# Lecanyu/SparsifyPoseGraph

Hardware: AMD Instinct MI355X
Metric: nodes_marginalized_per_s (higher is better)
Workload: dtype f64

## Files before the change

sparsifyposegraph_amd/csrc/spg_graph_impl.h:

```cpp
#pragma once
#include <algorithm>
#include <atomic>
#include <chrono>
#include <cmath>
#include <cstdio>
#include <cstdlib>
#include <cstring>
#include <set>
#include <string>
#include <thread>
#if defined(__linux__)
#include <pthread.h>
#include <sched.h>
#endif
#include <unistd.h>
#include <unordered_map>
#include <unordered_set>
#include <vector>
#include "../../include/spg.h"
#include "spg_internal.h"

namespace {
inline int pose_stride(int d) { return d == 3 ? 3 : 7; }
inline int info_len(int d) { return d * (d + 1) / 2; }
inline double now_s() {
    return std::chrono::duration<double>(std::chrono::steady_clock::now().time_since_epoch()).count();
}
inline int64_t align_up(int64_t x, int64_t a) { return (x + a - 1) / a * a; }
inline void cpu_pause() {
#if defined(__x86_64__)
    __builtin_ia32_pause();
#endif
}
inline void spin_wait(uint32_t &spins) {
    if (++spins > 4096) std::this_thread::yield();
    else cpu_pause();
}
}

struct HostMirror {
    double *p = nullptr;
    size_t n = 0, cap = 0;
    ~HostMirror() { free(p); }
    HostMirror() {}
    HostMirror(const HostMirror &) = delete;
    HostMirror &operator=(const HostMirror &) = delete;
    double *data() { return p; }
    const double *data() const { return p; }
    size_t size() const { return n; }
    double &operator[](size_t i) { return p[i]; }
    const double &operator[](size_t i) const { return p[i]; }
    void resize(size_t m) {
        if (m > cap) {
            size_t nc = std::max(m, cap * 2);
            p = (double *)realloc(p, nc * sizeof(double));
            if (!p) abort();
            cap = nc;
        }
        n = m;
    }
};

template <class T, int N>
struct InlVec {
    int32_t n = 0, cap = N;
    union { T inl[N]; T *ptr; };
    InlVec() {}
    InlVec(const InlVec &o) : n(o.n), cap(o.cap) {
        if (cap > N) { ptr = (T *)malloc(sizeof(T) * (size_t)cap); memcpy(ptr, o.ptr, sizeof(T) * (size_t)n); }
        else memcpy(inl, o.inl, sizeof inl);
    }
    InlVec(InlVec &&o) noexcept : n(o.n), cap(o.cap) {
        if (cap > N) { ptr = o.ptr; o.cap = N; o.n = 0; }
        else memcpy(inl, o.inl, sizeof inl);
    }
    InlVec &operator=(InlVec o) noexcept {
        if (cap > N) free(ptr);
        n = o.n; cap = o.cap;
        if (cap > N) { ptr = o.ptr; o.cap = N; o.n = 0; }
        else memcpy(inl, o.inl, sizeof inl);
        return *this;
    }
    ~InlVec() { if (cap > N) free(ptr); }
    T *data() { return cap > N ? ptr : inl; }
    const T *data() const { return cap > N ? ptr : inl; }
    T *begin() { return data(); }
    T *end() { return data() + n; }
    const T *begin() const { return data(); }
    const T *end() const { return data() + n; }
    size_t size() const { return (size_t)n; }
    bool empty() const { return n == 0; }
    T &operator[](size_t i) { return data()[i]; }
    const T &operator[](size_t i) const { return data()[i]; }
    T &back() { return data()[n - 1]; }
    void pop_back() { n--; }
    void clear() { n = 0; }
    void push_back(const T &v) {
        if (n == cap) {
            int32_t nc = cap * 2;
            T *p = (T *)malloc(sizeof(T) * (size_t)nc);
            if (!p) abort();
            memcpy(p, data(), sizeof(T) * (size_t)n);
            if (cap > N) free(ptr);
            ptr = p; cap = nc;
        }
        data()[n++] = v;
    }
};

struct spg_ctx {
    spg_backend be{};
    bool is_hip = false;
    int rank = 0, nranks = 1;
    void *rccl = nullptr;
    int tag_counter = 0;
    int linear_solver = 0;
    double pcg_rel_tol = 0;
    int pcg_max_iter = 0;
    spg_pcg_stats pcg_stats{};
    spg::StreamPort *sim_port = nullptr;
    char err[768] = {0};
};

struct GEdge {
    int64_t off;
    int64_t key;
    int32_t len;
    int32_t vtx[2];
    int16_t nv;
    int8_t kind;
    uint8_t alive;
};

struct RoundBlanket {
    int32_t root;
    int32_t n_remove;
    int32_t vbeg = 0, nv = 0;
    int32_t ebeg = 0, ne = 0;
    int32_t rank = 0;
    int32_t owner = -1;
    spg_blanket_desc desc{};
};

struct BlanketLog { int32_t root_id, round, status, info; double kld, min_gap; };

struct Batch {
    std::vector<RoundBlanket> rb;
    std::vector<int32_t> rb_verts, rb_edges;
    std::vector<spg_blanket_desc> h_blk;
    std::vector<int64_t> h_vpo;
    std::vector<spg_edge_ref> h_er;
    std::vector<int32_t> h_ev;
    std::vector<int64_t> chunk_hdr;
    spg_round_info rinfo{};
    bool round_open = false;
    bool used_mailbox = false;
    int eff_ranks = 1, eff_rank = 0;
    int slot = 0;
    int seq = 0;
    int round_no = 0;
    int tag = 0;
    double t_launch = 0;
    std::vector<std::pair<int32_t, int64_t>> kld_pending;
    alignas(64) std::atomic<int> submitted{1};
    int submit_rc = 0;
    char pad_[56];
};

struct OwnRefT { int32_t oid; uint32_t gen; };

struct spg_graph {
    spg_ctx *ctx = nullptr;
    int d = 0, ps = 0, rec = 0;
    std::vector<int32_t> vid;
    std::unordered_map<int32_t, int32_t> vidx;
    std::vector<int32_t> vdirect;
    bool vdirect_ok = true;
    int32_t index_of(int32_t id) const {
        if (vdirect_ok) return (id >= 0 && (size_t)id < vdirect.size()) ? vdirect[(size_t)id] : -1;
        auto it = vidx.find(id);
        return it == vidx.end() ? -1 : it->second;
    }
    std::vector<uint8_t> valive;
    std::vector<int64_t> vpose;
    struct AdjEnt { int32_t eid, other; operator int32_t() const { return eid; } };
    struct SVtx {
        int32_t nown;
        int32_t own[4];
        int32_t slot;
    };
    struct alignas(64) VRec {
        InlVec<AdjEnt, 7> adj;
        SVtx s;
        int32_t id, pad_;
        int64_t pose;
        char spare_[24];
        VRec() { s.nown = 0; s.slot = -1; id = 0; pad_ = 0; pose = 0; }
    };
    std::vector<VRec> vr;
    std::vector<InlVec<struct OwnRefT, 3>> vown;
    std::vector<int32_t> cst;
    std::vector<GEdge> edges;
    std::vector<int32_t> everts;
    int n_live_v = 0, n_live_e = 0;
    void *dev = nullptr;
    int64_t cap = 0, used = 0;
    HostMirror host;
    int64_t dev_synced = 0;
    int64_t stale_lo = 0, stale_hi = 0;
    bool active = false;
    spg_options opts{};
    int rank = 0, nranks = 1;
    std::vector<int32_t> pending;
    size_t pend_head = 0;
    std::vector<uint8_t> in_set;
    static constexpr int NB = 8;
    Batch bt[NB];
    Batch *B = &bt[0];
    struct Owner { int32_t batch, off, len; uint32_t gen; };
    using OwnRef = OwnRefT;
    std::vector<Owner> owners;
    std::vector<int32_t> owner_free, transient;
    std::vector<int32_t> Dpool;
    int shard_threshold = -1;
    int round_no = 0, launch_seq = 0;
    bool pipelined = false;
    spg_marg_stats stats{};
    double tr_age = 0, tr_wait = 0, tr_first = 0; long tr_n = 0;
    std::vector<BlanketLog> log;
    std::vector<double> hdr_buf;
    std::thread sub_thread;
    static constexpr uint32_t SUBQ = 8;
    bool sub_active = false;
    struct alignas(64) SubShared {
        alignas(64) std::atomic<uint32_t> tail{0};
        alignas(64) Batch *q[SUBQ] = {nullptr};
        alignas(64) std::atomic<uint32_t> head{0};
        alignas(64) double seconds = 0;
        alignas(64) std::atomic<bool> run{false};
        char pad_[64];
    } sub;
    std::vector<int32_t> live_rank;
    long n_mutations = 0, live_rank_stamp = -1;
    int64_t next_key = 0, key_base = 0;
    static constexpr int64_t kKeyStride = 65536;
    std::vector<int32_t> lpos;
    std::vector<int32_t> vstamp, estamp;
    int32_t stamp = 0;
    std::vector<int32_t> ocnt;
    std::vector<int32_t> lidx;
    std::vector<int32_t> s_newpending, s_B, s_centres, s_Dv, s_tmp, s_work, s_seen, s_hit, s_vix;
    std::vector<double> s_cost;
    std::vector<int> s_first;
    static constexpr int kSOwn = 4, kSMaxV = 16, kSMaxE = 44;
    struct SSlot {
        int32_t pos, root, nv, ne, n_new_max, tag, logi, bell;
        int32_t launched;
        int32_t npend, pend[3];
        int32_t mcell;
        int64_t new_off, out_off;
        int32_t verts[kSMaxV];
        int32_t edges[kSMaxE];
    };
    std::vector<SSlot> sslots;
    std::vector<int32_t> s_free, s_fifo, s_fin, s_woken, s_ready, wl_next, wl_stable, wl_done;
    int64_t unsorted_from = -1;
    bool layout_diverged = false;
    int stream_emulation = -1;
    int stream_disabled = 0;
    int robust_kind = 0, robust_gap = 1;
    double robust_delta = 1.0;
};

static inline const int32_t *edge_verts(const spg_graph *g, const GEdge &e) {
    return e.nv == 2 ? e.vtx : g->everts.data() + e.vtx[0];
}

inline int set_err(spg_ctx *c, int code, const char *fmt, const char *a = "") {
    if (c) snprintf(c->err, sizeof c->err, fmt, a);
    return code;
}

int sync_host(spg_graph *g);
int sync_device(spg_graph *g);
void canonicalize_edge_order(spg_graph *g);
#pragma GCC visibility push(hidden)
int arena_ensure(spg_graph *g, int64_t need);
int add_edge_idx(spg_graph *g, int kind, int nv, const int32_t *vix, int64_t off, int32_t len, int64_t key = -1);
void pose_compose(int d, const double *a, const double *b, double *o);
void pose_inverse(int d, const double *a, double *o);
void quiesce_submission(spg_graph *g);
int stream_marginalize(spg_graph *g, bool *started = nullptr);
#pragma GCC visibility pop

namespace {
inline void next_stamp(spg_graph *g) {
    if (g->vstamp.size() < g->vid.size()) g->vstamp.resize(g->vid.size(), 0);
    if (g->estamp.size() < g->edges.size()) g->estamp.resize(g->edges.size(), 0);
    g->stamp++;
}

inline void mark_stale(spg_graph *g, int64_t lo, int64_t hi) {
    if (g->stale_hi <= g->stale_lo) { g->stale_lo = lo; g->stale_hi = hi; }
    else { g->stale_lo = std::min(g->stale_lo, lo); g->stale_hi = std::max(g->stale_hi, hi); }
}

inline void copy_backend_error(spg_ctx *c) { snprintf(c->err, sizeof c->err, "%s", spg::hip_backend_error(&c->be)); }

enum MailState { MAIL_NOT_YET = 0, MAIL_READY = 1, MAIL_FINAL = 2 };
inline MailState mail_state(double word, double tag) {
    return word == SPG_READY_WORD(tag) ? MAIL_READY : word == SPG_FINAL_WORD(tag) ? MAIL_FINAL : MAIL_NOT_YET;
}

inline bool out_record_well_formed(const double *rec, const spg_blanket_desc &bd, int nv) {
    const int n_new = (int)rec[4];
    if (n_new < 0 || n_new > bd.n_new_max) return false;
    int vsum = 0;
    for (int e = 0; e < n_new; e++) {
        const double nvd = rec[SPG_OUT_HDR + 4 * e + 3], reld = rec[SPG_OUT_HDR + 4 * e + 1], lend = rec[SPG_OUT_HDR + 4 * e + 2];
        if (!(nvd >= 1 && nvd <= nv && reld >= 0 && lend >= 1 && reld + lend <= (double)bd.new_len)) return false;
        for (int i = 0; i < (int)nvd; i++) { const double li = rec[SPG_OUT_HDR + 4 * bd.n_new_max + vsum + i]; if (!(li >= 0 && li < nv)) return false; }
        vsum += (int)nvd;
        if (vsum > bd.n_new_vert_max) return false;
    }
    return true;
}
template <class F>
inline void for_each_new_edge(const double *rec, int n_new, int n_new_max, F &&fn) {
    const double *lv = rec + SPG_OUT_HDR + 4 * n_new_max;
    for (int e = 0; e < n_new; e++) {
        const double *t = rec + SPG_OUT_HDR + 4 * e;
        const int nv = (int)t[3];
        fn(e, (int)t[0], (int64_t)t[1], (int32_t)t[2], nv, lv);
        lv += nv;
    }
}
template <class F>
inline void for_each_compact_edge(const double *rec, int n_new, F &&fn) {
    uint64_t w[2];
    memcpy(w, rec + 6, 16);
    for (int e = 0; e < n_new; e++) {
        const unsigned pr = (unsigned)(w[e >> 3] >> (8 * (e & 7))) & 0xffu;
        fn(e, (int)(pr & 15u), (int)(pr >> 4));
    }
}

inline void new_edge_budget(const spg_options &o, int d, int k, int32_t &n_new_max, int32_t &n_new_vert_max, int64_t &new_len) {
    int ps = pose_stride(d);
    if (o.algorithm == SPG_ALG_NFR) {
        n_new_max = std::max(k - 1, 0);
        if (k > 2 && (o.topology == SPG_TOPO_DENSE || o.topology == SPG_TOPO_SUBGRAPH)) {
            const int msub = (int)((1 + o.chord_ratio) * (k - 1)), all = k * (k - 1) / 2;
            n_new_max = (o.topology == SPG_TOPO_DENSE || msub >= all) ? all : std::max(msub, k - 1);
        }
        n_new_vert_max = 2 * n_new_max;
        new_len = (int64_t)n_new_max * (ps + info_len(d));
        if (k > 2 && (o.topology == SPG_TOPO_CLIQUEY_SUBGRAPH || o.topology == SPG_TOPO_CLIQUEY_DENSE)) new_len += SPG_MULTI_LEN(d, k - 1);
    } else if (o.topology == SPG_TOPO_DENSE || k <= 1) {
        int64_t n = (int64_t)d * k;
        n_new_max = k > 0 ? 1 : 0;
        n_new_vert_max = k;
        new_len = n + n * n;
    } else {
        int64_t n2 = 2 * d;
        n_new_max = k;
        n_new_vert_max = 2 * k - 1;
        new_len = (d + (int64_t)d * d) + (int64_t)(k - 1) * (n2 + n2 * n2);
    }
}

inline void append_blanket_desc(spg_graph *g, const int32_t *verts, int nv, int n_remove, const int32_t *eids, int ne,
                                spg_blanket_desc &bd, std::vector<int64_t> &h_vpo, std::vector<spg_edge_ref> &h_er, std::vector<int32_t> &h_ev) {
    const int d = g->d;
    int32_t *const lidx = g->lidx.data();
    memset(&bd, 0, sizeof bd);
    bd.vert_begin = (int32_t)h_vpo.size();
    bd.n_vert = nv;
    bd.n_remove = n_remove;
    for (int i = 0; i < nv; i++) { h_vpo.push_back(g->vpose[verts[i]]); lidx[verts[i]] = (int32_t)i; }
    bd.edge_begin = (int32_t)h_er.size();
    bd.n_edge = ne;
    int32_t scratch = 0;
    for (int ei = 0; ei < ne; ei++) {
        const GEdge &e = g->edges[eids[ei]];
        if (e.kind == SPG_EDGE_GLC) scratch = std::max(scratch, e.len - d * e.nv + e.nv * 2 * d * d);
        spg_edge_ref er;
        er.off = e.off; er.len = e.len; er.kind = e.kind; er.vbegin = (int32_t)h_ev.size(); er.nv = e.nv;
        for (int i = 0; i < e.nv; i++) h_ev.push_back(lidx[edge_verts(g, e)[i]]);
        h_er.push_back(er);
    }
    bd.pad_ = scratch;
    bd.tinfo_off = -1;
}
}
```

sparsifyposegraph_amd/csrc/spg_host.cpp:

```cpp
#include "spg_graph_impl.h"

#if defined(__linux__)
#include <execinfo.h>
#include <signal.h>
#include <dlfcn.h>
static void spg_segv_handler(int sig) {
    void *frames[64];
    const int n = backtrace(frames, 64);
    Dl_info di;
    const char *base = nullptr;
    if (dladdr((void *)&spg_segv_handler, &di)) base = (const char *)di.dli_fbase;
    char line[160];
    int len = snprintf(line, sizeof line, "spg: signal %d; frames relative to libspg_hip.so (base %p):\n", sig, (const void *)base);
    if (write(2, line, (size_t)len) < 0) {}
    for (int i = 0; i < n; i++) {
        Dl_info fi;
        const bool ours = dladdr(frames[i], &fi) && fi.dli_fbase == (void *)base;
        len = snprintf(line, sizeof line, "  #%d %s0x%llx\n", i, ours ? "+" : "abs ", (unsigned long long)(ours ? (const char *)frames[i] - base : (const char *)frames[i] - (const char *)0));
        if (write(2, line, (size_t)len) < 0) {}
    }
    signal(sig, SIG_DFL);
    raise(sig);
}
static void spg_install_segv_trace() {
    static bool done = false;
    const char *e = getenv("SPG_SEGV_BACKTRACE");
    if (done || !(e && e[0] == '1')) return;
    done = true;
    signal(SIGSEGV, spg_segv_handler);
    signal(SIGABRT, spg_segv_handler);
}
#else
static void spg_install_segv_trace() {}
#endif

extern "C" int spg_ctx_create(spg_ctx **out, int device) {
    spg_install_segv_trace();
    if (!out) return SPG_EINVAL;
    spg_ctx *c = new spg_ctx;
    int rc = spg::hip_backend_create(device, &c->be, c->err, sizeof c->err);
    if (rc != 0) {
        fprintf(stderr, "libspg_hip: %s\n", c->err);
        delete c;
        *out = nullptr;
        return rc;
    }
    c->is_hip = true;
    *out = c;
    return 0;
}

extern "C" int spg_ctx_create_injected(spg_ctx **out, const spg_backend *backend) {
    if (!out || !backend || !backend->alloc || !backend->run_round) return SPG_EINVAL;
    spg_ctx *c = new spg_ctx;
    c->be = *backend;
    c->is_hip = false;
    *out = c;
    return 0;
}

extern "C" int spg_get_unique_id(void *id_out) {
    if (!id_out) return SPG_EINVAL;
    char err[256];
    int rc = spg::rccl_get_unique_id(id_out, err, sizeof err);
    if (rc) fprintf(stderr, "libspg_hip: %s\n", err);
    return rc;
}

extern "C" int spg_ctx_create_ranks(spg_ctx **out, int device, int rank, int nranks, const void *nccl_unique_id) {
    if (!out || nranks < 1 || rank < 0 || rank >= nranks) return SPG_EINVAL;
    int rc = spg_ctx_create(out, device);
    if (rc) return rc;
    spg_ctx *c = *out;
    c->rank = rank; c->nranks = nranks;
    if (nccl_unique_id) {
        rc = spg::rccl_comm_create(device, rank, nranks, nccl_unique_id, &c->rccl, c->err, sizeof c->err);
        if (rc) {
            fprintf(stderr, "libspg_hip: %s\n", c->err);
            spg_ctx_destroy(c);
            *out = nullptr;
            return rc;
        }
    }
    return 0;
}
extern "C" int spg_ctx_set_linear_solver(spg_ctx *c, int solver) {
    if (!c || solver < SPG_SOLVER_AUTO || solver > SPG_SOLVER_PCG) return SPG_EINVAL;
    c->linear_solver = solver;
    return 0;
}
extern "C" int spg_ctx_set_pcg(spg_ctx *c, double rel_tol, int max_iter) {
    if (!c || std::isnan(rel_tol)) return SPG_EINVAL;
    c->pcg_rel_tol = rel_tol > 0 ? rel_tol : 0;
    c->pcg_max_iter = max_iter > 0 ? max_iter : 0;
    return 0;
}
extern "C" int spg_ctx_set_factor_descent(spg_ctx *c, double rel_tol, int max_cycles) {
    if (!c || std::isnan(rel_tol) || max_cycles > 32767) return SPG_EINVAL;
    const int cycles = max_cycles > 0 ? max_cycles : spg::kFdMaxCycles;
    const double tol = rel_tol > 0 ? rel_tol : (rel_tol == 0 && max_cycles > 0) ? 0.0 : spg::kFdRelTol;
    if (c->is_hip) spg::hip_backend_set_factor_descent(&c->be, tol, cycles);
    return 0;
}
extern "C" int spg_ctx_pcg_stats(spg_ctx *c, spg_pcg_stats *out) {
    if (!c || !out) return SPG_EINVAL;
    *out = c->pcg_stats;
    return 0;
}

extern "C" int spg_ctx_rank(const spg_ctx *c) { return c ? c->rank : 0; }
extern "C" int spg_ctx_nranks(const spg_ctx *c) { return c ? c->nranks : 0; }

extern "C" int spg_allgather_region(spg_ctx *c, void *arena, int64_t region_off, int64_t chunk_len) {
    if (!c || !arena || region_off < 0 || chunk_len < 0) return SPG_EINVAL;
    if (!c->rccl) {
        if (c->nranks > 1) return set_err(c, SPG_ESTATE, "spg_allgather_region: the context has %s ranks but no RCCL communicator (spg_ctx_create_ranks without a unique id)", std::to_string(c->nranks).c_str());
        return 0;
    }
    return spg::rccl_allgather_f64(c->rccl, arena, region_off, chunk_len, spg::hip_backend_stream(&c->be), c->err, sizeof c->err);
}

extern "C" void spg_ctx_destroy(spg_ctx *c) {
    if (!c) return;
    if (c->rccl) spg::rccl_comm_destroy(c->rccl);
    if (c->is_hip) spg::hip_backend_destroy(&c->be);
    delete c;
}
extern "C" void spg_free(void *p) { free(p); }

extern "C" const char *spg_last_error(spg_ctx *c) {
    if (!c) return "";
    if (c->err[0]) return c->err;
    return c->is_hip ? spg::hip_backend_error(&c->be) : "";
}
extern "C" void *spg_ctx_stream(spg_ctx *c) { return (c && c->is_hip) ? spg::hip_backend_stream(&c->be) : nullptr; }
extern "C" int spg_ctx_synchronize(spg_ctx *c) { return c ? c->be.synchronize(c->be.user) : SPG_EINVAL; }

extern "C" int spg_ctx_profile(spg_ctx *c, int enable) {
    if (!c || !c->is_hip) return SPG_EINVAL;
    spg::hip_backend_profile(&c->be, enable);
    return 0;
}
extern "C" int spg_ctx_profile_read_worker(spg_ctx *c, double *kernel_ms, double *alg_bytes, int64_t *runs, int64_t *blankets) {
    if (!c || !c->is_hip || !kernel_ms || !alg_bytes || !runs || !blankets) return SPG_EINVAL;
    long long r = 0, b = 0;
    spg::hip_backend_profile_read_worker(&c->be, kernel_ms, alg_bytes, &r, &b);
    *runs = r; *blankets = b;
    return 0;
}
extern "C" int spg_ctx_profile_read_big(spg_ctx *c, double *kernel_ms, double *flops, int64_t *blankets, int32_t *n_max) {
    if (!c || !c->is_hip || !kernel_ms || !flops || !blankets || !n_max) return SPG_EINVAL;
    long long cnt = 0;
    int nm = 0;
    spg::hip_backend_profile_read_big(&c->be, kernel_ms, flops, &cnt, &nm);
    *blankets = cnt; *n_max = nm;
    return 0;
}
extern "C" int spg_ctx_profile_read(spg_ctx *c, double *kernel_ms, double *alg_bytes, int64_t *launches, int64_t *blankets) {
    if (!c || !c->is_hip || !kernel_ms || !alg_bytes || !launches || !blankets) return SPG_EINVAL;
    long long l = 0, b = 0;
    spg::hip_backend_profile_read(&c->be, kernel_ms, alg_bytes, &l, &b);
    *launches = l; *blankets = b;
    return 0;
}

static int emit(const std::vector<int> &v, int32_t *out, int cap) {
    for (size_t i = 0; i < v.size() && (int)i < cap; i++) out[i] = v[i];
    return (int)v.size();
}
extern "C" int spg_decimate_cluster(int last, int endvert, int sparsity, int clusterSize, int32_t *out, int cap) {
    std::vector<int> ret;
    if (clusterSize > 0 && (((last - 4) % clusterSize == 0 && last > 4) || last == endvert)) {
        for (int i = int(std::ceil((last - 5) / (double)clusterSize) - 1) * clusterSize + 5; i <= last; i++)
            if (i % sparsity > 0) ret.push_back(i);
    }
    return emit(ret, out, cap);
}
extern "C" int spg_decimate_online(int last, int, int sparsity, int, int32_t *out, int cap) {
    std::vector<int> ret;
    if (last % sparsity != 0) ret.push_back(last);
    return emit(ret, out, cap);
}
extern "C" int spg_decimate_global(int last, int endvert, int sparsity, int, int32_t *out, int cap) {
    std::vector<int> ret;
    if (last == endvert)
        for (int i = 4; i <= endvert; i++)
            if (i % sparsity != 0) ret.push_back(i);
    return emit(ret, out, cap);
}

int sync_host(spg_graph *g) {
    if (g->stale_hi > g->stale_lo) {
        if ((int64_t)g->host.size() < g->used) g->host.resize((size_t)g->used);
        int rc = g->ctx->be.download(g->ctx->be.user, g->host.data() + g->stale_lo,
                                     (char *)g->dev + g->stale_lo * 8, g->stale_hi - g->stale_lo);
        if (rc) return rc;
        g->stale_lo = g->stale_hi = 0;
    }
    return 0;
}

int sync_device(spg_graph *g) {
    if (g->dev_synced < g->used) {
        if (int rc = arena_ensure(g, g->used)) return rc;
        int64_t lo = g->dev_synced;
        int rc = g->ctx->be.upload(g->ctx->be.user, (char *)g->dev + lo * 8, g->host.data() + lo, g->used - lo);
        if (rc) return rc;
        g->dev_synced = g->used;
    }
    return 0;
}

int arena_ensure(spg_graph *g, int64_t need) {
    if (need <= g->cap && g->dev) return 0;
    if (int rc = sync_host(g)) return rc;
    int64_t nc = std::max<int64_t>(need, std::max<int64_t>(g->cap * 2, 1 << 16));
    void *nd = g->ctx->be.alloc(g->ctx->be.user, nc);
    if (!nd) return set_err(g->ctx, SPG_ENOMEM, "arena allocation failed");
    if (g->dev) g->ctx->be.release(g->ctx->be.user, g->dev);
    g->dev = nd;
    g->cap = nc;
    g->dev_synced = 0;
    if ((int64_t)g->host.size() < g->used) g->host.resize((size_t)g->used);
    return 0;
}

static int64_t arena_push(spg_graph *g, const double *src, int64_t len) {
    int64_t off = g->used;
    if ((int64_t)g->host.size() < off + len) g->host.resize((size_t)std::max<int64_t>(off + len, (int64_t)g->host.size() * 2));
    if (src) memcpy(g->host.data() + off, src, (size_t)len * 8);
    g->used += len;
    return off;
}

extern "C" int spg_graph_create(spg_ctx *ctx, int pose_dim, spg_graph **out) {
    if (!ctx || !out || (pose_dim != 3 && pose_dim != 6)) return SPG_EINVAL;
    spg_graph *g = new spg_graph;
    g->ctx = ctx;
    g->d = pose_dim;
    g->ps = pose_stride(pose_dim);
    g->rec = g->ps + info_len(pose_dim);
    *out = g;
    return 0;
}

extern "C" void spg_graph_destroy(spg_graph *g) {
    if (!g) return;
    if (g->dev) g->ctx->be.release(g->ctx->be.user, g->dev);
    delete g;
}

extern "C" int spg_graph_add_vertex(spg_graph *g, int id, const double *pose) {
    if (!g || !pose || g->active) return SPG_EINVAL;
    if (g->vidx.count(id)) return set_err(g->ctx, SPG_EINVAL, "duplicate vertex id");
    int32_t idx = (int32_t)g->vid.size();
    g->vid.push_back(id);
    g->vidx[id] = idx;
    if (g->vdirect_ok) {
        if (id < 0 || (size_t)id > 8 * g->vid.size() + 4096) { g->vdirect_ok = false; g->vdirect.clear(); g->vdirect.shrink_to_fit(); }
        else { if ((size_t)id >= g->vdirect.size()) g->vdirect.resize(std::max<size_t>((size_t)id + 1, g->vdirect.size() * 2), -1); g->vdirect[(size_t)id] = idx; }
    }
    g->valive.push_back(1);
    g->vr.emplace_back();
    g->vown.emplace_back();
    g->vpose.push_back(arena_push(g, pose, g->ps));
    g->vr.back().id = id;
    g->vr.back().pose = g->vpose.back();
    g->n_live_v++;
    return 0;
}

int add_edge_idx(spg_graph *g, int kind, int nv, const int32_t *vix, int64_t off, int32_t len, int64_t key) {
    if (g->sub_active && (g->edges.size() == g->edges.capacity() || (nv != 2 && g->everts.size() + (size_t)nv > g->everts.capacity()))) {
        quiesce_submission(g);
        g->edges.reserve(std::max<size_t>(g->edges.capacity() * 2, 1024));
        g->everts.reserve(std::max<size_t>(g->everts.capacity() * 2 + (size_t)nv, 1024));
    }
    GEdge e;
    e.kind = (int8_t)kind; e.nv = (int16_t)nv; e.len = len; e.off = off; e.alive = 1;
    e.key = key >= 0 ? key : g->next_key++;
    if (nv == 2) { e.vtx[0] = vix[0]; e.vtx[1] = vix[1]; }
    else { e.vtx[0] = (int32_t)g->everts.size(); e.vtx[1] = 0; }
    int32_t eid = (int32_t)g->edges.size();
    if (nv != 2) for (int i = 0; i < nv; i++) g->everts.push_back(vix[i]);
    g->edges.push_back(e);
    g->n_mutations++;
    for (int i = 0; i < nv; i++) {
        bool dup = false;
        for (int j = 0; j < i; j++) dup |= (vix[j] == vix[i]);
        if (!dup) g->vr[vix[i]].adj.push_back({eid, (nv == 2 && kind == SPG_EDGE_BINARY) ? vix[1 - i] : -1});
    }
    g->n_live_e++;
    return eid;
}

extern "C" int spg_graph_add_edge(spg_graph *g, int from, int to, const double *meas, const double *info_upper) {
    if (!g || !meas || !info_upper || g->active) return SPG_EINVAL;
    auto a = g->vidx.find(from), b = g->vidx.find(to);
    if (a == g->vidx.end() || b == g->vidx.end() || !g->valive[a->second] || !g->valive[b->second])
        return set_err(g->ctx, SPG_EINVAL, "edge endpoint does not exist");
    int64_t off = arena_push(g, meas, g->ps);
    arena_push(g, info_upper, info_len(g->d));
    int32_t vix[2] = {a->second, b->second};
    add_edge_idx(g, SPG_EDGE_BINARY, 2, vix, off, g->rec);
    return 0;
}

extern "C" int spg_graph_add_glc_edge(spg_graph *g, int q, const int32_t *ids, int r, const double *meas, const double *W) {
    if (!g || q < 1 || r < 1 || !ids || !meas || !W || g->active) return SPG_EINVAL;
    std::vector<int32_t> vix(q);
    for (int i = 0; i < q; i++) {
        auto it = g->vidx.find(ids[i]);
        if (it == g->vidx.end() || !g->valive[it->second]) return set_err(g->ctx, SPG_EINVAL, "edge endpoint does not exist");
        vix[i] = it->second;
    }
    int n = g->d * q;
    int64_t off = arena_push(g, meas, n);
    arena_push(g, W, (int64_t)r * n);
    add_edge_idx(g, SPG_EDGE_GLC, q, vix.data(), off, n + r * n);
    return 0;
}

extern "C" int spg_graph_add_multi_edge(spg_graph *g, int q, const int32_t *ids, const double *record, int64_t len) {
    if (!g || q < 2 || !ids || !record || g->active) return SPG_EINVAL;
    const int nm = (int)record[0];
    if (nm < 1 || len != SPG_MULTI_LEN(g->d, nm)) return set_err(g->ctx, SPG_EINVAL, "multi edge record length does not match its measurement count");
    for (int i = 0; i < 2 * nm; i++) if (record[1 + i] < 0 || record[1 + i] >= q) return set_err(g->ctx, SPG_EINVAL, "multi edge: a measurement refers to a vertex outside the edge");
    std::vector<int32_t> vix(q);
    for (int i = 0; i < q; i++) {
        auto it = g->vidx.find(ids[i]);
        if (it == g->vidx.end() || !g->valive[it->second]) return set_err(g->ctx, SPG_EINVAL, "edge endpoint does not exist");
        vix[i] = it->second;
    }
    int64_t off = arena_push(g, record, len);
    add_edge_idx(g, SPG_EDGE_MULTI, q, vix.data(), off, (int32_t)len);
    return 0;
}

extern "C" int spg_graph_add_vertices(spg_graph *g, int n, const int32_t *ids, const double *poses) {
    if (!g || n < 0 || !ids || !poses) return SPG_EINVAL;
    g->vid.reserve(g->vid.size() + n);
    for (int i = 0; i < n; i++)
        if (int rc = spg_graph_add_vertex(g, ids[i], poses + (size_t)i * g->ps)) return rc;
    return 0;
}
extern "C" int spg_graph_add_edges(spg_graph *g, int n, const int32_t *ij, const double *records) {
    if (!g || n < 0 || !ij || !records) return SPG_EINVAL;
    g->edges.reserve(g->edges.size() + n);
    for (int i = 0; i < n; i++) {
        const double *r = records + (size_t)i * g->rec;
        if (int rc = spg_graph_add_edge(g, ij[2 * i], ij[2 * i + 1], r, r + g->ps)) return rc;
    }
    return 0;
}

extern "C" int spg_graph_pose_dim(const spg_graph *g) { return g ? g->d : 0; }
extern "C" int spg_graph_num_vertices(const spg_graph *g) { return g ? g->n_live_v : 0; }
extern "C" int spg_graph_num_edges(const spg_graph *g) { return g ? g->n_live_e : 0; }
void canonicalize_edge_order(spg_graph *g) {
    if (g->unsorted_from < 0 || g->active) return;
    const size_t from = (size_t)g->unsorted_from, n = g->edges.size() - from;
    g->unsorted_from = -1;
    if (n < 2) return;
    std::vector<uint32_t> perm(n);
    for (size_t i = 0; i < n; i++) perm[i] = (uint32_t)i;
    bool sorted = true;
    for (size_t i = 1; i < n && sorted; i++) sorted = g->edges[from + i - 1].key <= g->edges[from + i].key;
    if (sorted) return;
    std::stable_sort(perm.begin(), perm.end(), [&](uint32_t a, uint32_t b) { return g->edges[from + a].key < g->edges[from + b].key; });
    std::vector<int32_t> newid(n);
    std::vector<GEdge> tmp(n);
    for (size_t i = 0; i < n; i++) { tmp[i] = g->edges[from + perm[i]]; newid[perm[i]] = (int32_t)(from + i); }
    std::copy(tmp.begin(), tmp.end(), g->edges.begin() + (long)from);
    next_stamp(g);
    const int32_t st = g->stamp;
    for (size_t i = 0; i < n; i++) {
        const GEdge &e = g->edges[from + i];
        if (!e.alive) continue;
        for (int t = 0; t < e.nv; t++) {
            const int32_t v = edge_verts(g, e)[t];
            if (g->vstamp[v] == st) continue;
            g->vstamp[v] = st;
            for (auto &a : g->vr[v].adj) if ((size_t)a.eid >= from) a.eid = newid[(size_t)a.eid - from];
        }
    }
    g->n_mutations++;
}

extern "C" int64_t spg_graph_edge_data_size(const spg_graph *g) {
    int64_t s = 0;
    for (auto &e : g->edges) if (e.alive) s += e.len;
    return s;
}
extern "C" int64_t spg_graph_edge_vert_size(const spg_graph *g) {
    int64_t s = 0;
    for (auto &e : g->edges) if (e.alive) s += e.nv;
    return s;
}

extern "C" int spg_graph_get_vertices(spg_graph *g, int32_t *ids, double *poses) {
    if (!g) return SPG_EINVAL;
    if (int rc = sync_host(g)) return rc;
    std::vector<std::pair<int32_t, int32_t>> order;
    for (size_t i = 0; i < g->vid.size(); i++) if (g->valive[i]) order.push_back({g->vid[i], (int32_t)i});
    std::sort(order.begin(), order.end());
    for (size_t k = 0; k < order.size(); k++) {
        ids[k] = order[k].first;
        memcpy(poses + k * g->ps, g->host.data() + g->vpose[order[k].second], (size_t)g->ps * 8);
    }
    return (int)order.size();
}

extern "C" int spg_graph_get_edges(spg_graph *g, int32_t *kind, int32_t *vert_off, int32_t *vert_ids, int64_t *data_off, double *data) {
    if (!g) return SPG_EINVAL;
    canonicalize_edge_order(g);
    if (int rc = sync_host(g)) return rc;
    int ne = 0, nv = 0;
    int64_t nd = 0;
    vert_off[0] = 0; data_off[0] = 0;
    for (auto &e : g->edges) {
        if (!e.alive) continue;
        kind[ne] = e.kind;
        for (int i = 0; i < e.nv; i++) vert_ids[nv++] = g->vid[edge_verts(g, e)[i]];
        memcpy(data + nd, g->host.data() + e.off, (size_t)e.len * 8);
        nd += e.len;
        ne++;
        vert_off[ne] = nv; data_off[ne] = nd;
    }
    return ne;
}

extern "C" int spg_graph_set_estimate(spg_graph *g, int id, const double *pose) {
    if (!g || !pose || g->active) return SPG_EINVAL;
    auto it = g->vidx.find(id);
    if (it == g->vidx.end() || !g->valive[it->second]) return SPG_EINVAL;
    int64_t off = g->vpose[it->second];
    memcpy(g->host.data() + off, pose, (size_t)g->ps * 8);
    if (off < g->dev_synced && g->dev)
        return g->ctx->be.upload(g->ctx->be.user, (char *)g->dev + off * 8, pose, g->ps);
    return 0;
}

extern "C" void *spg_graph_arena(spg_graph *g, int64_t *capacity) {
    if (!g) return nullptr;
    if (capacity) *capacity = g->cap;
    return g->dev;
}

extern "C" int spg_graph_reserve(spg_graph *g, int64_t arena_doubles) {
    if (!g) return SPG_EINVAL;
    if (int rc = arena_ensure(g, std::max(arena_doubles, g->used))) return rc;
    if ((int64_t)g->host.size() < g->cap) g->host.resize((size_t)g->cap);
    {
        const size_t ne = g->edges.size(), nl = g->log.size();
        g->edges.resize(2 * ne + 1024); g->edges.resize(ne);
        g->log.resize(g->vid.size() + 16); g->log.resize(nl);
        auto touch = [](auto &v, size_t n) { if (v.capacity() < n) { const size_t keep = v.size(); v.resize(n); v.resize(keep); } };
        const size_t nv = g->vid.size();
        for (int i = 0; i < spg_graph::NB; i++) {
            Batch &b = g->bt[i];
            touch(b.rb, 1024); touch(b.rb_verts, 16384); touch(b.rb_edges, 32768); touch(b.h_blk, 1024); touch(b.h_vpo, 16384);
            touch(b.h_er, 32768); touch(b.h_ev, 65536); touch(b.kld_pending, 1024);
        }
        touch(g->pending, nv); touch(g->in_set, nv); touch(g->vstamp, nv); touch(g->estamp, 2 * ne + 1024);
        touch(g->owners, 8192); touch(g->ocnt, 8192); touch(g->owner_free, 8192); touch(g->transient, 4096); touch(g->Dpool, 65536);
        touch(g->s_newpending, 4096); touch(g->hdr_buf, 65536);
    }
    return sync_device(g);
}

static void normalize_quat(double *q) {
    double n = std::sqrt(q[0] * q[0] + q[1] * q[1] + q[2] * q[2] + q[3] * q[3]);
    if (n > 0) for (int i = 0; i < 4; i++) q[i] /= n;
}

extern "C" int spg_graph_load_g2o(spg_ctx *ctx, const char *path, spg_graph **out) {
    if (!ctx || !path || !out) return SPG_EINVAL;
    FILE *f = fopen(path, "r");
    if (!f) return set_err(ctx, SPG_EIO, "cannot open %s", path);
    struct V { int id; double p[7]; };
    struct E { int a, b; double r[28]; };
    struct GE { std::vector<int32_t> ids; int r = 0, n = 0; std::vector<double> meas, W; };
    std::vector<V> vs;
    std::vector<E> es;
    std::vector<GE> ges;
    int d = 0;
    char *lbuf = nullptr;
    size_t lcap = 0;
    bool bad_glc = false, has_multi = false;
    while (getline(&lbuf, &lcap, f) >= 0) {
        char *s = lbuf;
        while (*s == ' ' || *s == '\t') s++;
        char tag[64];
        int adv = 0;
        if (sscanf(s, "%63s%n", tag, &adv) != 1) continue;
        s += adv;
        auto readn = [&](double *dst, int cnt) {
            for (int i = 0; i < cnt; i++) {
                char *end;
                dst[i] = strtod(s, &end);
                if (end == s) return false;
                s = end;
            }
            return true;
        };
        auto readi = [&](int &v) {
            char *end;
            long x = strtol(s, &end, 10);
            if (end == s) return false;
            v = (int)x; s = end;
            return true;
        };
        if (!strcmp(tag, "VERTEX_SE2")) {
            V v{};
            if (!readi(v.id) || !readn(v.p, 3)) continue;
            if (!d) d = 3;
            vs.push_back(v);
        } else if (!strcmp(tag, "VERTEX_SE3:QUAT")) {
            V v{};
            if (!readi(v.id) || !readn(v.p, 7)) continue;
            normalize_quat(v.p + 3);
            if (!d) d = 6;
            vs.push_back(v);
        } else if (!strcmp(tag, "EDGE_SE2")) {
            E e{};
            if (!readi(e.a) || !readi(e.b) || !readn(e.r, 9)) continue;
            es.push_back(e);
        } else if (!strcmp(tag, "EDGE_SE3:QUAT")) {
            E e{};
            if (!readi(e.a) || !readi(e.b) || !readn(e.r, 28)) continue;
            normalize_quat(e.r + 3);
            es.push_back(e);
        } else if (!strcmp(tag, "GLC_EDGE")) {
            GE ge;
            for (;;) {
                while (*s == ' ' || *s == '\t') s++;
                if (s[0] == '|' && s[1] == '|') { s += 2; break; }
                int id;
                if (!readi(id)) { bad_glc = true; break; }
                ge.ids.push_back(id);
            }
            char rtag[64];
            int adv2 = 0;
            if (bad_glc || sscanf(s, "%63s%n", rtag, &adv2) != 1) { bad_glc = true; continue; }
            s += adv2;
            if (!readi(ge.r) || !readi(ge.n) || ge.r < 1 || ge.n < 1 || ge.ids.empty() || ge.n % (int)ge.ids.size()) { bad_glc = true; continue; }
            ge.meas.resize(ge.n);
            ge.W.resize((size_t)ge.r * ge.n);
            std::vector<double> info((size_t)ge.r * (ge.r + 1) / 2);
            if (!readn(ge.meas.data(), ge.n) || !readn(ge.W.data(), ge.r * ge.n) || !readn(info.data(), (int)info.size())) { bad_glc = true; continue; }
            bool ident = true;
            {
                size_t p2 = 0;
                for (int i = 0; i < ge.r; i++) for (int j = i; j < ge.r; j++) { ident &= (info[p2] == (i == j ? 1.0 : 0.0)); p2++; }
            }
            if (!ident) {
                std::vector<double> Lm((size_t)ge.r * ge.r, 0.0);
                size_t p2 = 0;
                for (int i = 0; i < ge.r; i++) for (int j = i; j < ge.r; j++) { Lm[(size_t)j * ge.r + i] = info[p2]; p2++; }
                bool pd = true;
                for (int j = 0; j < ge.r && pd; j++) {
                    double dj = Lm[(size_t)j * ge.r + j];
                    for (int k = 0; k < j; k++) dj -= Lm[(size_t)j * ge.r + k] * Lm[(size_t)j * ge.r + k];
                    if (!(dj > 0)) { pd = false; break; }
                    double l = std::sqrt(dj);
                    Lm[(size_t)j * ge.r + j] = l;
                    for (int i = j + 1; i < ge.r; i++) {
                        double sacc = Lm[(size_t)i * ge.r + j];
                        for (int k = 0; k < j; k++) sacc -= Lm[(size_t)i * ge.r + k] * Lm[(size_t)j * ge.r + k];
                        Lm[(size_t)i * ge.r + j] = sacc / l;
                    }
                }
                if (!pd) { bad_glc = true; continue; }
                std::vector<double> W2((size_t)ge.r * ge.n, 0.0);
                for (int i = 0; i < ge.r; i++) for (int k = i; k < ge.r; k++) for (int c = 0; c < ge.n; c++) W2[(size_t)i * ge.n + c] += Lm[(size_t)k * ge.r + i] * ge.W[(size_t)k * ge.n + c];
                ge.W.swap(W2);
            }
            ges.push_back(std::move(ge));
        } else if (!strncmp(tag, "MULTI_EDGE_", 11)) {
            has_multi = true;
        }
    }
    free(lbuf);
    fclose(f);
    if (has_multi) return set_err(ctx, SPG_EIO, "%s holds MULTI_EDGE_* records: that format omits the vertex pair of each measurement and cannot be read back", path);
    if (bad_glc) return set_err(ctx, SPG_EIO, "malformed GLC_EDGE record in %s", path);
    if (!d) return set_err(ctx, SPG_EIO, "no SE2/SE3 vertices in %s", path);
    std::stable_sort(vs.begin(), vs.end(), [](const V &a, const V &b) { return a.id < b.id; });
    spg_graph *g;
    if (int rc = spg_graph_create(ctx, d, &g)) return rc;
    for (auto &v : vs) if (int rc = spg_graph_add_vertex(g, v.id, v.p)) { spg_graph_destroy(g); return rc; }
    for (auto &e : es) if (int rc = spg_graph_add_edge(g, e.a, e.b, e.r, e.r + g->ps)) { spg_graph_destroy(g); return rc; }
    for (auto &ge : ges) {
        if (ge.n != d * (int)ge.ids.size()) { spg_graph_destroy(g); return set_err(ctx, SPG_EIO, "GLC_EDGE dimension does not match its vertices in %s", path); }
        if (int rc = spg_graph_add_glc_edge(g, (int)ge.ids.size(), ge.ids.data(), ge.r, ge.meas.data(), ge.W.data())) { spg_graph_destroy(g); return rc; }
    }
    *out = g;
    return 0;
}

static void write_g2o_stream(spg_graph *g, FILE *f);
extern "C" int spg_graph_write_g2o(spg_graph *g, const char *path) {
    if (!g || !path) return SPG_EINVAL;
    if (int rc = sync_host(g)) return rc;
    FILE *f = fopen(path, "w");
    if (!f) return set_err(g->ctx, SPG_EIO, "cannot open %s for writing", path);
    write_g2o_stream(g, f);
    fclose(f);
    return 0;
}
extern "C" int spg_graph_write_g2o_mem(spg_graph *g, char **text, size_t *len) {
    if (!g || !text || !len) return SPG_EINVAL;
    if (int rc = sync_host(g)) return rc;
    *text = nullptr; *len = 0;
    FILE *f = open_memstream(text, len);
    if (!f) return set_err(g->ctx, SPG_ENOMEM, "open_memstream failed");
    write_g2o_stream(g, f);
    fclose(f);
    return 0;
}
static void write_g2o_stream(spg_graph *g, FILE *f) {
    canonicalize_edge_order(g);
    std::vector<std::pair<int32_t, int32_t>> order;
    for (size_t i = 0; i < g->vid.size(); i++) if (g->valive[i]) order.push_back({g->vid[i], (int32_t)i});
    std::sort(order.begin(), order.end());
    const char *vt = g->d == 3 ? "VERTEX_SE2" : "VERTEX_SE3:QUAT", *et = g->d == 3 ? "EDGE_SE2" : "EDGE_SE3:QUAT";
    for (auto &o : order) {
        fprintf(f, "%s %d", vt, o.first);
        for (int i = 0; i < g->ps; i++) fprintf(f, " %.17g", g->host[g->vpose[o.second] + i]);
        fputc('\n', f);
    }
    for (auto &e : g->edges) {
        if (!e.alive) continue;
        if (e.kind == SPG_EDGE_BINARY) {
            fprintf(f, "%s %d %d", et, g->vid[edge_verts(g, e)[0]], g->vid[edge_verts(g, e)[1]]);
            for (int i = 0; i < e.len; i++) fprintf(f, " %.17g", g->host[e.off + i]);
        } else if (e.kind == SPG_EDGE_MULTI) {
            const double *rec = g->host.data() + e.off;
            const int nm = (int)rec[0], r = g->d * nm;
            const double *meas = rec + 1 + 2 * nm, *W = meas + (size_t)nm * g->ps;
            fprintf(f, "%s", g->d == 3 ? "MULTI_EDGE_SE2" : "MULTI_EDGE_SE3");
            for (int i = 0; i < e.nv; i++) fprintf(f, " %d", g->vid[edge_verts(g, e)[i]]);
            fprintf(f, " || %d %d", nm, g->ps);
            for (int i = 0; i < nm * g->ps; i++) fprintf(f, " %.17g", meas[i]);
            for (int i = 0; i < r; i++) for (int j = i; j < r; j++) {
                double v = 0;
                for (int t = 0; t < r; t++) v += W[(size_t)t * r + i] * W[(size_t)t * r + j];
                fprintf(f, " %.17g", v);
            }
        } else {
            int n = g->d * e.nv, r = (e.len - n) / n;
            fprintf(f, "GLC_EDGE");
            for (int i = 0; i < e.nv; i++) fprintf(f, " %d", g->vid[edge_verts(g, e)[i]]);
            fprintf(f, " || %s %d %d", g->d == 3 ? "GLC_REPARAM_SE2_ISAM" : "GLC_REPARAM_SE3", r, n);
            for (int i = 0; i < e.len; i++) fprintf(f, " %.17g", g->host[e.off + i]);
            for (int i = 0; i < r; i++) for (int j = i; j < r; j++) fprintf(f, " %d", i == j ? 1 : 0);
        }
        fputc('\n', f);
    }
}

extern "C" int spg_graph_clone_portion(spg_graph *g, int maxid, spg_graph **out) {
    if (!g || !out || g->active) return SPG_EINVAL;
    canonicalize_edge_order(g);
    if (int rc = sync_host(g)) return rc;
    spg_graph *c;
    if (int rc = spg_graph_create(g->ctx, g->d, &c)) return rc;
    std::vector<std::pair<int32_t, int32_t>> order;
    for (size_t i = 0; i < g->vid.size(); i++) if (g->valive[i] && g->vid[i] <= maxid) order.push_back({g->vid[i], (int32_t)i});
    std::sort(order.begin(), order.end());
    int rc = 0;
    for (auto &o : order) if ((rc = spg_graph_add_vertex(c, o.first, g->host.data() + g->vpose[o.second]))) break;
    std::vector<int32_t> ids;
    for (size_t ei = 0; ei < g->edges.size() && !rc; ei++) {
        const GEdge &e = g->edges[ei];
        if (!e.alive) continue;
        bool in = true;
        ids.clear();
        for (int i = 0; i < e.nv; i++) { int32_t id = g->vid[edge_verts(g, e)[i]]; in &= (id <= maxid); ids.push_back(id); }
        if (!in) continue;
        const double *rec = g->host.data() + e.off;
        if (e.kind == SPG_EDGE_BINARY) rc = spg_graph_add_edge(c, ids[0], ids[1], rec, rec + g->ps);
        else if (e.kind == SPG_EDGE_MULTI) rc = spg_graph_add_multi_edge(c, e.nv, ids.data(), rec, e.len);
        else { int n = g->d * e.nv; rc = spg_graph_add_glc_edge(c, e.nv, ids.data(), (e.len - n) / n, rec, rec + n); }
    }
    if (rc) { spg_graph_destroy(c); return rc; }
    c->robust_kind = g->robust_kind; c->robust_delta = g->robust_delta; c->robust_gap = g->robust_gap;
    *out = c;
    return 0;
}

extern "C" int spg_graph_vertex_edges(spg_graph *g, int id, int32_t *edge_index, int cap) {
    if (!g || (cap > 0 && !edge_index)) return SPG_EINVAL;
    auto it = g->vidx.find(id);
    if (it == g->vidx.end() || !g->valive[it->second]) return set_err(g->ctx, SPG_EINVAL, "no such vertex");
    std::vector<int32_t> es(g->vr[it->second].adj.begin(), g->vr[it->second].adj.end());
    std::sort(es.begin(), es.end());
    if (g->live_rank_stamp != g->n_mutations || g->live_rank.size() != g->edges.size()) {
        g->live_rank.resize(g->edges.size());
        int32_t r = 0;
        for (size_t e = 0; e < g->edges.size(); e++) { g->live_rank[e] = r; r += g->edges[e].alive ? 1 : 0; }
        g->live_rank_stamp = g->n_mutations;
    }
    int n = 0;
    for (int32_t e : es) { if (n < cap) edge_index[n] = g->live_rank[e]; n++; }
    return n;
}

extern "C" int spg_debug_la(int op, int M, int N, int K, int flags, int mode, double *A, int ra, int lda, double *B, int rb, int ldb, double *C, int rc, int ldc, int *ok) {
    if (!A || !B || !C || !ok || M <= 0 || lda <= 0 || ldb <= 0 || ldc <= 0) return SPG_EINVAL;
    return spg::hip_la_test(op, M, N, K, flags, mode, A, ra, lda, B, rb, ldb, C, rc, ldc, ok);
}

extern "C" int spg_graph_last_blanket_count(const spg_graph *g) { return g ? (int)g->log.size() : 0; }
extern "C" int spg_graph_last_blankets(const spg_graph *g, int32_t *root_id, int32_t *round, int32_t *status, int32_t *info, double *kld, double *min_gap) {
    if (!g) return SPG_EINVAL;
    for (size_t i = 0; i < g->log.size(); i++) {
        if (root_id) root_id[i] = g->log[i].root_id;
        if (round) round[i] = g->log[i].round;
        if (status) status[i] = g->log[i].status;
        if (info) info[i] = g->log[i].info;
        if (kld) kld[i] = g->log[i].kld;
        if (min_gap) min_gap[i] = g->log[i].min_gap;
    }
    return (int)g->log.size();
}

extern "C" int spg_marginalize_batch(spg_ctx *ctx, const spg_options *o, const spg_batch *bt, spg_result *r) {
    if (!ctx || !o || !bt || !r) return SPG_EINVAL;
    const int d = o->pose_dim;
    if (d != 3 && d != 6) return SPG_EINVAL;
    const int ps = pose_stride(d);
    const int B = bt->B;
    r->new_edge_off[0] = 0;
    r->new_edge_vert_off[0] = 0;
    r->new_edge_data_off[0] = 0;
    if (B == 0) return 0;
    const int V = bt->vert_off[B], E = bt->edge_off[B];
    const int64_t ED = bt->edge_data_off[E];
    std::vector<double> host;
    int64_t o_pose = 0, o_edge = (int64_t)V * ps;
    int64_t cur = align_up(o_edge + ED, 32);
    std::vector<spg_blanket_desc> blk(B);
    std::vector<int64_t> vpo(V);
    std::vector<spg_edge_ref> er(E);
    for (int v = 0; v < V; v++) vpo[v] = o_pose + (int64_t)v * ps;
    for (int e = 0; e < E; e++) {
        er[e].off = o_edge + bt->edge_data_off[e];
        er[e].len = (int32_t)(bt->edge_data_off[e + 1] - bt->edge_data_off[e]);
        er[e].kind = bt->edge_kind[e];
        er[e].vbegin = bt->edge_vert_off[e];
        er[e].nv = bt->edge_vert_off[e + 1] - bt->edge_vert_off[e];
    }
    for (int b = 0; b < B; b++) {
        spg_blanket_desc &bd = blk[b];
        memset(&bd, 0, sizeof bd);
        bd.vert_begin = bt->vert_off[b];
        bd.n_vert = bt->vert_off[b + 1] - bt->vert_off[b];
        bd.n_remove = bt->n_remove[b];
        bd.edge_begin = bt->edge_off[b];
        bd.n_edge = bt->edge_off[b + 1] - bt->edge_off[b];
        int k = bd.n_vert - bd.n_remove;
        new_edge_budget(*o, d, std::max(k, 0), bd.n_new_max, bd.n_new_vert_max, bd.new_len);
        for (int e = bd.edge_begin; e < bd.edge_begin + bd.n_edge; e++)
            if (er[e].kind == SPG_EDGE_GLC) bd.pad_ = std::max(bd.pad_, er[e].len - d * er[e].nv + er[e].nv * 2 * d * d);
        bd.out_off = cur; cur += SPG_OUT_LEN(bd.n_new_max, bd.n_new_vert_max);
        bd.new_off = cur; cur += bd.new_len;
        if (r->target_info) { int64_t n = (int64_t)d * std::max(k, 0); bd.tinfo_off = cur; cur += n * n; }
        else bd.tinfo_off = -1;
    }
    int64_t in_len = align_up(o_edge + ED, 32);
    host.assign((size_t)cur, 0.0);
    memcpy(host.data(), bt->pose, (size_t)V * ps * 8);
    if (ED) memcpy(host.data() + o_edge, bt->edge_data, (size_t)ED * 8);
    void *dev = ctx->be.alloc(ctx->be.user, cur);
    if (!dev) return set_err(ctx, SPG_ENOMEM, "arena allocation failed");
    int rc = ctx->be.upload(ctx->be.user, dev, host.data(), in_len);
    spg_round_desc rd{};
    rd.opts = o;
    rd.n_blankets = B; rd.first = 0; rd.count = B;
    rd.blankets = blk.data();
    rd.vert_pose_off = vpo.data();
    rd.edges = er.data();
    rd.edge_vert = bt->edge_vert;
    rd.n_vert_total = V; rd.n_edge_total = E; rd.n_edge_vert_total = bt->edge_vert_off[E];
    if (!rc) rc = ctx->be.run_round(ctx->be.user, dev, &rd);
    if (!rc) rc = ctx->be.synchronize(ctx->be.user);
    if (!rc && cur > in_len) rc = ctx->be.download(ctx->be.user, host.data() + in_len, (char *)dev + in_len * 8, cur - in_len);
    ctx->be.release(ctx->be.user, dev);
    if (rc) {
        if (ctx->is_hip) copy_backend_error(ctx);
        return rc;
    }
    int32_t ne = 0, nev = 0;
    int64_t ned = 0;
    for (int b = 0; b < B; b++) {
        const spg_blanket_desc &bd = blk[b];
        const double *rec = host.data() + bd.out_off;
        r->status[b] = (int32_t)rec[0];
        if (r->info) r->info[b] = (int32_t)rec[1];
        r->kld[b] = rec[2];
        if (r->min_gap) r->min_gap[b] = rec[3];
        int n_new = (int)rec[4];
        int k = bd.n_vert - bd.n_remove;
        if (r->target_info && k > 0) {
            int64_t n = (int64_t)d * k;
            memcpy(r->target_info + r->target_info_off[b], host.data() + bd.tinfo_off, (size_t)(n * n) * 8);
        }
        int vpos = 0;
        for (int e = 0; e < n_new; e++) {
            int kind = (int)rec[SPG_OUT_HDR + 4 * e + 0];
            int64_t rel = (int64_t)rec[SPG_OUT_HDR + 4 * e + 1];
            int64_t len = (int64_t)rec[SPG_OUT_HDR + 4 * e + 2];
            int nv = (int)rec[SPG_OUT_HDR + 4 * e + 3];
            if (ne + 1 > r->new_edge_cap || nev + nv > r->new_edge_vert_cap || ned + len > r->new_edge_data_cap) return SPG_ECAPACITY;
            r->new_edge_kind[ne] = kind;
            for (int i = 0; i < nv; i++)
                r->new_edge_vert[nev++] = bt->vert_id[bd.vert_begin + (int)rec[SPG_OUT_HDR + 4 * bd.n_new_max + vpos + i]];
            vpos += nv;
            memcpy(r->new_edge_data + ned, host.data() + bd.new_off + rel, (size_t)len * 8);
            ned += len;
            ne++;
            r->new_edge_vert_off[ne] = nev;
            r->new_edge_data_off[ne] = ned;
        }
        r->new_edge_off[b + 1] = ne;
    }
    return 0;
}

namespace {
struct HPose { double t[3]; double q[4]; double th; };

void q_mul(const double *a, const double *b, double *o) {
    o[0] = a[3] * b[0] + a[0] * b[3] + a[1] * b[2] - a[2] * b[1];
    o[1] = a[3] * b[1] - a[0] * b[2] + a[1] * b[3] + a[2] * b[0];
    o[2] = a[3] * b[2] + a[0] * b[1] - a[1] * b[0] + a[2] * b[3];
    o[3] = a[3] * b[3] - a[0] * b[0] - a[1] * b[1] - a[2] * b[2];
}
void q_rot(const double *q, const double *v, double *o) {
    double x = q[0], y = q[1], z = q[2], w = q[3];
    double tx = 2 * (y * v[2] - z * v[1]), ty = 2 * (z * v[0] - x * v[2]), tz = 2 * (x * v[1] - y * v[0]);
    o[0] = v[0] + w * tx + (y * tz - z * ty);
    o[1] = v[1] + w * ty + (z * tx - x * tz);
    o[2] = v[2] + w * tz + (x * ty - y * tx);
}
double wrap_theta(double th) {
    const double PI = 3.14159265358979323846;
    if (th >= -PI && th < PI) return th;
    double m = std::fmod(th, 2 * PI);
    if (m >= PI) m -= 2 * PI;
    if (m < -PI) m += 2 * PI;
    return m;
}
}
void pose_compose(int d, const double *a, const double *b, double *o) {
    if (d == 3) {
        double c = std::cos(a[2]), s = std::sin(a[2]);
        o[0] = a[0] + c * b[0] - s * b[1]; o[1] = a[1] + s * b[0] + c * b[1]; o[2] = wrap_theta(a[2] + b[2]);
    } else {
        double r[3];
        q_rot(a + 3, b, r);
        o[0] = a[0] + r[0]; o[1] = a[1] + r[1]; o[2] = a[2] + r[2];
        q_mul(a + 3, b + 3, o + 3);
        double n = std::sqrt(o[3] * o[3] + o[4] * o[4] + o[5] * o[5] + o[6] * o[6]);
        for (int i = 3; i < 7; i++) o[i] /= n;
    }
}
void pose_inverse(int d, const double *a, double *o) {
    if (d == 3) {
        double c = std::cos(a[2]), s = std::sin(a[2]);
        o[0] = -(c * a[0] + s * a[1]); o[1] = -(-s * a[0] + c * a[1]); o[2] = wrap_theta(-a[2]);
    } else {
        double qi[4] = {-a[3], -a[4], -a[5], a[6]}, r[3];
        q_rot(qi, a, r);
        o[0] = -r[0]; o[1] = -r[1]; o[2] = -r[2];
        o[3] = qi[0]; o[4] = qi[1]; o[5] = qi[2]; o[6] = qi[3];
    }
}
namespace {
bool dense_inverse(int n, std::vector<double> &A) {
    std::vector<double> X((size_t)n * n, 0.0);
    for (int i = 0; i < n; i++) X[(size_t)i * n + i] = 1.0;
    for (int k = 0; k < n; k++) {
        int p = k;
        for (int i = k + 1; i < n; i++) if (std::fabs(A[(size_t)i * n + k]) > std::fabs(A[(size_t)p * n + k])) p = i;
        if (A[(size_t)p * n + k] == 0.0) return false;
        if (p != k) for (int j = 0; j < n; j++) { std::swap(A[(size_t)k * n + j], A[(size_t)p * n + j]); std::swap(X[(size_t)k * n + j], X[(size_t)p * n + j]); }
        double ip = 1.0 / A[(size_t)k * n + k];
        for (int j = 0; j < n; j++) { A[(size_t)k * n + j] *= ip; X[(size_t)k * n + j] *= ip; }
        for (int i = 0; i < n; i++) {
            if (i == k) continue;
            double f = A[(size_t)i * n + k];
            if (f == 0.0) continue;
            for (int j = 0; j < n; j++) { A[(size_t)i * n + j] -= f * A[(size_t)k * n + j]; X[(size_t)i * n + j] -= f * X[(size_t)k * n + j]; }
        }
    }
    A.swap(X);
    return true;
}
}

extern "C" int spg_graph_substitute_edge(spg_graph *g, const int32_t *marginalized, int n_marg, int maxid,
                                         int *from, int *to, double *meas, double *info_upper) {
    if (!g || !from || !to || !meas || !info_upper || (n_marg > 0 && !marginalized)) return SPG_EINVAL;
    if (int rc = sync_host(g)) return rc;
    const int d = g->d, ps = g->ps;
    const size_t NV = g->vid.size();
    auto slot_of = [&](int id) -> int32_t { auto it = g->vidx.find(id); return (it == g->vidx.end() || !g->valive[it->second]) ? -1 : it->second; };
    const int id_new = std::max(*from, *to), id_gone = std::min(*from, *to);
    const int32_t s_new = slot_of(id_new), s_gone = slot_of(id_gone);
    if (s_new < 0 || s_gone < 0) return set_err(g->ctx, SPG_EINVAL, "substitute edge endpoint does not exist");
    std::vector<uint8_t> flag(NV, 0);
    for (int i = 0; i < n_marg; i++) { int32_t sl = slot_of(marginalized[i]); if (sl >= 0) flag[sl] |= 1; }
    std::vector<int32_t> level, lvl_off{0}, nextl;
    level.push_back(s_gone);
    lvl_off.push_back(1);
    flag[s_new] |= 2; flag[s_gone] |= 2;
    int32_t hit = -1;
    for (;;) {
        const int32_t lo = lvl_off[lvl_off.size() - 2], hi = lvl_off.back();
        nextl.clear();
        for (int32_t p = lo; p < hi; p++) {
            const int32_t v = level[p];
            const int id = g->vid[v];
            if (!(flag[v] & 1) && id != *from && id != *to) {
                if (hit < 0 || id < g->vid[hit]) hit = v;
                continue;
            }
            flag[v] |= 2;
            for (int32_t eid : g->vr[v].adj) {
                const GEdge &e = g->edges[eid];
                if (e.nv != 2) continue;
                const int32_t u = (e.vtx[0] == v) ? e.vtx[1] : e.vtx[0];
                if ((flag[u] & 2) || g->vid[u] > maxid || g->vid[u] == 0 || (flag[u] & 4)) continue;
                flag[u] |= 4;
                nextl.push_back(u);
            }
        }
        if (hit >= 0) break;
        if (nextl.empty()) return set_err(g->ctx, SPG_EINVAL, "no surviving vertex reachable");
        std::sort(nextl.begin(), nextl.end(), [&](int32_t a, int32_t b) { return g->vid[a] < g->vid[b]; });
        for (int32_t u : nextl) flag[u] &= (uint8_t)~4;
        level.insert(level.end(), nextl.begin(), nextl.end());
        lvl_off.push_back((int32_t)level.size());
    }
    const int n_levels = (int)lvl_off.size() - 1;
    std::vector<double> cov((size_t)d * d, 0.0), acc(ps, 0.0), nxt(ps), zinv(ps), om((size_t)d * d);
    if (d == 6) acc[6] = 1.0;
    std::vector<uint8_t> in_prev(NV, 0);
    std::vector<int32_t> es;
    int32_t cur = hit;
    const bool new_is_from = (*from == id_new);
    for (int l = n_levels - 2; l >= -1; l--) {
        if (l >= 0) for (int32_t p = lvl_off[l]; p < lvl_off[l + 1]; p++) in_prev[level[p]] = 1;
        else in_prev[s_new] = 1;
        es.assign(g->vr[cur].adj.begin(), g->vr[cur].adj.end());
        std::sort(es.begin(), es.end());
        bool stepped = false;
        for (int32_t eid : es) {
            const GEdge &e = g->edges[eid];
            if (e.nv != 2 || e.kind != SPG_EDGE_BINARY) continue;
            if (!(in_prev[e.vtx[0]] || in_prev[e.vtx[1]])) continue;
            const double *rec = g->host.data() + e.off;
            int q = 0;
            for (int i = 0; i < d; i++) for (int j = i; j < d; j++) { om[(size_t)i * d + j] = om[(size_t)j * d + i] = rec[ps + q]; q++; }
            if (!dense_inverse(d, om)) return set_err(g->ctx, SPG_EINVAL, "singular edge information on the substitute path");
            for (int i = 0; i < d * d; i++) cov[i] += om[i];
            const bool cur_is_head = (e.vtx[1] == cur);
            if (new_is_from) {
                if (cur_is_head) pose_compose(d, rec, acc.data(), nxt.data());
                else { pose_inverse(d, rec, zinv.data()); pose_compose(d, zinv.data(), acc.data(), nxt.data()); }
            } else {
                if (cur_is_head) { pose_inverse(d, rec, zinv.data()); pose_compose(d, acc.data(), zinv.data(), nxt.data()); }
                else pose_compose(d, acc.data(), rec, nxt.data());
            }
            acc.swap(nxt);
            cur = cur_is_head ? e.vtx[0] : e.vtx[1];
            stepped = true;
            break;
        }
        if (l >= 0) for (int32_t p = lvl_off[l]; p < lvl_off[l + 1]; p++) in_prev[level[p]] = 0;
        else in_prev[s_new] = 0;
        (void)stepped;
    }
    if (!dense_inverse(d, cov)) return set_err(g->ctx, SPG_EINVAL, "singular covariance sum");
    int q = 0;
    for (int i = 0; i < d; i++) for (int j = i; j < d; j++) info_upper[q++] = 0.5 * (cov[(size_t)i * d + j] + cov[(size_t)j * d + i]);
    for (int i = 0; i < ps; i++) meas[i] = acc[i];
    if (new_is_from) *to = g->vid[hit]; else *from = g->vid[hit];
    return 0;
}
```

sparsifyposegraph_amd/csrc/spg_host_stream.cpp:

```cpp
#include "spg_graph_impl.h"

#if defined(__x86_64__)
#include <x86intrin.h>
static inline uint64_t ticks_now() { return __rdtsc(); }
#else
static inline uint64_t ticks_now() { return (uint64_t)(now_s() * 1e9); }
#endif

namespace {
enum : uint8_t { SV_WAITING = 0, SV_STABLE = 1, SV_INFLIGHT = 2, SV_DONE = 3 };
constexpr int kStreamSlots = 2048;
constexpr int kStreamMailStride = 8;

__attribute__((always_inline)) inline void unregister_blanket(spg_graph *g, const int32_t s) {
    const spg_graph::SSlot &sl = g->sslots[s];
    spg_graph::VRec *const vr = g->vr.data();
    for (int i = 0; i < sl.nv; i++) {
        spg_graph::SVtx &sx = vr[sl.verts[i]].s;
        for (int j = 0; j < sx.nown; j++) if (sx.own[j] == s) { sx.own[j] = sx.own[--sx.nown]; break; }
    }
}

struct Streamer {
    spg_graph *g;
    const bool emulate;
    const int D, ps, rec;
    const int32_t P;
    int32_t cursor = 0;
    int32_t prefetched_to = 0;
    int32_t n_done = 0, n_inflight = 0, pending_bell = 0, bell_no = 0;
    bool fallback = false;
    int32_t cap_wait = -1;
    uint64_t t_idle = 0;

    Streamer(spg_graph *g_, bool emu) : g(g_), emulate(emu), D(g_->d), ps(g_->ps), rec(g_->rec), P((int32_t)g_->pending.size()), arena_dev(g_->dev) {}

    struct SvView { spg_graph::VRec *vr; spg_graph::SVtx &operator[](int32_t i) const { return vr[i].s; } };

    long n_exam = 0, n_park[8] = {0};
    const bool prof = [] { const char *e = getenv("SPG_STREAM_PROF"); return e && e[0] == '1'; }();
    uint64_t pt[8] = {0}, pn[8] = {0}, pt_last = 0;
    inline void P0() { if (prof) pt_last = ticks_now(); }
    inline void P1(int i) { if (prof) { const uint64_t n = ticks_now(); pt[i] += n - pt_last; pn[i]++; pt_last = n; } }
    void park(std::vector<int32_t> &heads, int32_t on, int32_t p) { g->wl_next[p] = heads[on]; heads[on] = p; }
    void wake(std::vector<int32_t> &heads, int32_t on) {
        for (int32_t p = heads[on]; p >= 0;) { const int32_t nx = g->wl_next[p]; g->s_woken.push_back(p); p = nx; }
        heads[on] = -1;
    }

    static inline int find(const int32_t *X, const int nX, const int32_t y) { for (int i = 0; i < nX; i++) if (X[i] == y) return i; return -1; }
    static inline void adj_remove(InlVec<spg_graph::AdjEnt, 7> &av, const int32_t eid) {
        for (size_t j = 0; j < av.size(); j++) if (av[j].eid == eid) { av[j] = av.back(); av.pop_back(); break; }
    }
    inline void set_pend(spg_graph::SSlot &sl, const int32_t *X, const int nX) {
        const int32_t *const cst = g->cst.data();
        sl.npend = 0;
        for (int i = 1; i < nX; i++) if (cst[X[i]] >= 0) { if (sl.npend == 3) { sl.npend = -1; break; } sl.pend[sl.npend++] = X[i]; }
    }
    __attribute__((always_inline)) inline void register_blanket(const int32_t s, const int32_t p, const int32_t *X, const int nX) {
        const SvView sv{g->vr.data()};
        spg_graph::SSlot &sl = g->sslots[s];
        sl.pos = p; sl.root = X[0]; sl.nv = nX;
        memcpy(sl.verts, X, sizeof(int32_t) * (size_t)nX);
        set_pend(sl, X, nX);
        for (int i = 0; i < nX; i++) { spg_graph::SVtx &sx = sv[X[i]]; sx.own[sx.nown++] = s; }
    }

    void reserve(const int32_t p, const int32_t *X, const int nX) {
        const SvView sv{g->vr.data()};
        const int32_t v = X[0];
        if ((g->cst[v] & 3) != SV_WAITING || g->s_free.size() < 64) return;
        for (int i = 0; i < nX; i++) if (sv[X[i]].nown == spg_graph::kSOwn) return;
        const int32_t s = g->s_free.back(); g->s_free.pop_back();
        spg_graph::SSlot &sl = g->sslots[s];
        register_blanket(s, p, X, nX);
        sl.ne = 0; sl.launched = 0; sl.logi = -1;
        g->cst[v] = (p << 2) | SV_STABLE; sv[v].slot = s;
        if (g->wl_stable[p] >= 0) wake(g->wl_stable, p);
    }

    int examine(const int32_t p) {
        P0();
        const int r = examine_impl(p);
        P1(r ? 7 : 2);
        return r;
    }
    int examine_impl(const int32_t p) {
        const SvView sv{g->vr.data()};
        int32_t *const cst = g->cst.data();
        const int32_t v = g->pending[p];
        const int vstate = cst[v] & 3;
        if (vstate != SV_WAITING && vstate != SV_STABLE) return 0;
        n_exam++;
        spg_graph::VRec *const vr = g->vr.data();
        const GEdge *const edges = g->edges.data();
        const spg_graph::SSlot *const slots = g->sslots.data();
        int32_t X[spg_graph::kSMaxV];
        int nX = 1;
        int32_t mine = -1;
        if (vstate == SV_STABLE) {
            mine = sv[v].slot;
            nX = slots[mine].nv;
            memcpy(X, slots[mine].verts, sizeof(int32_t) * (size_t)nX);
        } else {
            X[0] = v;
            for (const spg_graph::AdjEnt &a : vr[v].adj) {
                const int32_t u = a.other;
                if (u < 0) { fallback = true; return 0; }
                if (find(X, nX, u) < 0) {
                    if (nX == spg_graph::kSMaxV) { fallback = true; return 0; }
                    X[nX++] = u;
                }
            }
            const int k0 = nX - 1;
            if (k0 < 1 || D * k0 > spg::kWorkerMaxN) { fallback = true; return 0; }
            int32_t blocker = -1;
            for (int i = 1; i < nX; i++) {
                const int32_t c = cst[X[i]];
                if (c >= 0 && (c & 3) != SV_DONE && ((c >> 2) < p || (c & 3) == SV_INFLIGHT)) blocker = std::max(blocker, c >> 2);
            }
            if (blocker >= 0) {
                n_park[0]++;
                park(g->wl_done, blocker, p);
                if (p >= prefetched_to) {
                    prefetched_to = p + 1;
                    __builtin_prefetch((const char *)&vr[v] + 64);
                    for (const spg_graph::AdjEnt &a : vr[v].adj) {
                        __builtin_prefetch(&edges[a.eid]);
                        __builtin_prefetch(&vr[a.other]);
                        __builtin_prefetch((const char *)&vr[a.other] + 64);
                    }
                }
                return 0;
            }
            for (int i = 2; i < nX; i++) {
                const int32_t x = X[i], idx = vr[x].id;
                int j = i - 1;
                for (; j >= 1 && vr[X[j]].id > idx; j--) X[j + 1] = X[j];
                X[j + 1] = x;
            }
        }
        const int k = nX - 1;
        for (int j = 0; j < sv[v].nown; j++) if (sv[v].own[j] != mine) { n_park[1]++; park(g->wl_done, slots[sv[v].own[j]].pos, p); return 0; }
        int32_t hs[spg_graph::kSMaxV * spg_graph::kSOwn];
        int nh = 0;
        for (int i = 1; i < nX; i++) {
            const spg_graph::SVtx &sx = sv[X[i]];
            for (int j = 0; j < sx.nown; j++) {
                const int32_t s = sx.own[j];
                if (s == mine) continue;
                if (!slots[s].launched && slots[s].pos > p) continue;
                for (int h = 0; h < nh; h++) if (hs[h] == s) { n_park[2]++; reserve(p, X, nX); park(g->wl_done, slots[s].pos, p); return 0; }
                hs[nh++] = s;
            }
        }
        {
            int32_t blocker = -1;
            for (int h = 0; h < nh; h++) {
                const spg_graph::SSlot &o = slots[hs[h]];
                if (o.pos > p) continue;
                const int32_t *mem = o.npend >= 0 ? o.pend : o.verts + 1;
                const int nmem = o.npend >= 0 ? o.npend : o.nv - 1;
                for (int i = 0; i < nmem; i++) {
                    const int32_t c = cst[mem[i]];
                    if (c >= 0 && (c & 3) == SV_WAITING && (c >> 2) < p) { blocker = std::max(blocker, o.pos); break; }
                }
            }
            if (blocker >= 0) { n_park[3]++; reserve(p, X, nX); park(g->wl_done, blocker, p); return 0; }
        }
        int32_t E[spg_graph::kSMaxE];
        int ne = 0;
        for (int i = 1; i < nX; i++) {
            for (const spg_graph::AdjEnt &a : vr[X[i]].adj) {
                const int32_t y = a.other;
                if (y < 0) { fallback = true; return 0; }
                const int j = find(X, nX, y);
                if (j >= 0) {
                    if (j == 0 || j >= i) {
                        if (ne == spg_graph::kSMaxE) { fallback = true; return 0; }
                        E[ne++] = a.eid;
                    }
                } else {
                    const int32_t c = cst[y];
                    if (c >= 0 && (c & 3) == SV_WAITING && (c >> 2) < p) { n_park[4]++; reserve(p, X, nX); park(g->wl_stable, c >> 2, p); return 0; }
                }
            }
        }
        const int words = spg::kPktHdr + nX + 4 * ne;
        if (words > spg::kPktWords) { fallback = true; return 0; }
        if (mine < 0) {
            for (int i = 0; i < nX; i++) if (sv[X[i]].nown == spg_graph::kSOwn) { park(g->wl_done, slots[sv[X[i]].own[0]].pos, p); return 0; }
            if (g->s_free.empty()) { g->wl_next[p] = cap_wait; cap_wait = p; return 0; }
        }
        if (!emulate && cell_slot[launch_seq & (uint32_t)(port.slots - 1)] != -1) { g->wl_next[p] = cap_wait; cap_wait = p; return 0; }
        const int n_new_max = k - 1, n_new_vert_max = 2 * (k - 1);
        const int64_t new_len = (int64_t)n_new_max * rec, out_len = emulate ? SPG_OUT_LEN(n_new_max, n_new_vert_max) : 0;
        if (g->used + new_len + out_len > g->cap) { fallback = true; return 0; }
        for (int i = 1; i < ne; i++) {
            const int32_t eid = E[i]; const int64_t key = edges[eid].key;
            int j = i - 1;
            for (; j >= 0 && edges[E[j]].key > key; j--) E[j + 1] = E[j];
            E[j + 1] = eid;
        }
        int32_t s = mine;
        if (s < 0) { s = g->s_free.back(); g->s_free.pop_back(); }
        spg_graph::SSlot &sl = g->sslots[s];
        if (mine < 0) register_blanket(s, p, X, nX);
        sl.ne = ne; sl.n_new_max = n_new_max; sl.logi = -1; sl.bell = bell_no + 1; sl.launched = 1;
        sl.tag = (++g->ctx->tag_counter & 0x3fffffff) + 1;
        sl.mcell = (int32_t)(launch_seq & (uint32_t)(port.slots - 1));
        if (!emulate) { cell_slot[sl.mcell] = s; launch_seq++; }
        sl.out_off = emulate ? g->used : -1;
        sl.new_off = g->used + out_len;
        g->used += new_len + out_len;
        memcpy(sl.edges, E, sizeof(int32_t) * (size_t)ne);
        cst[v] = (p << 2) | SV_INFLIGHT; sv[v].slot = s;
        P1(3);
        if (!emulate) build_packet(s, pending_bell);
        if (helper) hp.cell_tag[sl.mcell] = (uint32_t)sl.tag;
        P1(4);
        pending_bell++;
        n_inflight++;
        if (emulate) g->s_fifo.push_back(s);
        if (g->wl_stable[p] >= 0) wake(g->wl_stable, p);
        return 1;
    }

    void commit(const int32_t s, const double *recd, const bool final_seen) {
        spg_graph::SSlot &sl = g->sslots[s];
        const int32_t p = sl.pos, v = sl.root;
        const int status = (int)recd[0], inf = (int)recd[1], n_new = (int)recd[4];
        sl.logi = (int32_t)g->log.size();
        g->log.push_back({g->vid[v], sl.bell, status, inf, recd[2], recd[3]});
        g->stats.max_blanket = std::max(g->stats.max_blanket, sl.nv);
        const bool fine = (status == SPG_OK || status == SPG_ST_KLD_NOT_PD);
        if (!fine) g->stats.n_bad_status++;
        else {
            for (int i = 0; i < sl.ne; i++) {
                const int32_t eid = sl.edges[i];
                GEdge &e = g->edges[eid];
                e.alive = 0;
                adj_remove(g->vr[e.vtx[0]].adj, eid);
                if (e.vtx[1] != e.vtx[0]) adj_remove(g->vr[e.vtx[1]].adj, eid);
            }
            g->n_mutations += sl.ne + 1;
            g->n_live_e -= sl.ne;
            g->valive[v] = 0;
            g->vr[v].adj.clear();
            g->n_live_v--;
            g->stats.n_removed++;
            const int64_t key0 = g->key_base + (int64_t)p * spg_graph::kKeyStride;
            if (!emulate) {
                for_each_compact_edge(recd, n_new, [&](int e, int la, int lb) {
                    const int32_t va = sl.verts[la], vb = sl.verts[lb];
                    GEdge ge;
                    ge.off = sl.new_off + (int64_t)e * rec; ge.key = key0 + e; ge.len = rec; ge.vtx[0] = va; ge.vtx[1] = vb; ge.nv = 2; ge.kind = SPG_EDGE_BINARY; ge.alive = 1;
                    const int32_t eid = (int32_t)g->edges.size();
                    g->edges.push_back(ge);
                    g->vr[va].adj.push_back({eid, vb});
                    if (vb != va) g->vr[vb].adj.push_back({eid, va});
                });
            } else {
                for_each_new_edge(recd, n_new, sl.n_new_max, [&](int e, int kind, int64_t rel, int32_t len, int, const double *lv) {
                    int32_t vix[2] = {sl.verts[(int)lv[0]], sl.verts[(int)lv[1]]};
                    add_edge_idx(g, kind, 2, vix, sl.new_off + rel, len, key0 + e);
                });
            }
            g->stats.n_new_edges += n_new;
            if (!emulate) { g->n_mutations += n_new; g->n_live_e += n_new; }
        }
        unregister_blanket(g, s);
        g->cst[v] = (p << 2) | SV_DONE;
        n_done++;
        n_inflight--;
        if (final_seen) harvest(s, recd);
        else g->s_fin.push_back(s);
        if (g->wl_done[p] >= 0) wake(g->wl_done, p);
    }
    void harvest(const int32_t s, const double *recd) {
        spg_graph::SSlot &sl = g->sslots[s];
        BlanketLog &lg = g->log[sl.logi];
        lg.kld = recd[2]; lg.min_gap = recd[3]; lg.status = (int32_t)recd[0];
        if (std::isfinite(recd[2])) g->stats.kld_sum += recd[2];
        if (!emulate) cell_slot[sl.mcell] = -1;
        g->s_free.push_back(s);
        for (int32_t q = cap_wait; q >= 0;) { const int32_t nx = g->wl_next[q]; g->s_woken.push_back(q); q = nx; }
        cap_wait = -1;
    }

    alignas(64) spg::StreamPort port;
    void *arena_dev;
    static_assert(sizeof(spg::StreamPort) + sizeof(void *) == 64, "port + arena_dev = the cache line the poll helper reads");
    uint32_t launch_seq = 0, poll_seq = 0;
    std::vector<int32_t> cell_slot;
    double alg_bytes = 0;

    void build_packet(const int32_t s, const int ahead) {
        const spg_graph::SSlot &sl = g->sslots[s];
        const spg_graph::VRec *const vr = g->vr.data();
        const GEdge *const edges = g->edges.data();
        const int nX = sl.nv, ne = sl.ne, n_new_max = sl.n_new_max;
        const int words = spg::kPktHdr + nX + 4 * ne;
        unsigned long long pkt[spg::kPktWords];
        auto pack = [](int lo, int hi) { return (unsigned long long)(uint32_t)lo | ((unsigned long long)(uint32_t)hi << 32); };
        const spg_options &o = g->opts;
        pkt[0] = (unsigned long long)(uintptr_t)arena_dev;
        pkt[1] = port.d_mail;
        pkt[2] = 0;
        pkt[3] = (unsigned long long)((int64_t)sl.mcell * port.mail_stride); pkt[4] = (unsigned long long)sl.new_off; pkt[5] = (unsigned long long)(int64_t)-1;
        pkt[6] = pack(nX, 1); pkt[7] = pack(ne, n_new_max); pkt[8] = pack(2 * n_new_max, 0);
        pkt[9] = pack(o.topology, o.flags | (1 << 20)); pkt[10] = pack(o.lin_point, sl.tag);
        memcpy(&pkt[11], &o.chord_ratio, 8);
        pkt[12] = pack(words, 2 * ne);
        int w = spg::kPktHdr;
        for (int i = 0; i < nX; i++) pkt[w++] = (unsigned long long)vr[sl.verts[i]].pose;
        int32_t *evp = (int32_t *)(pkt + spg::kPktHdr + nX + 3 * ne);
        double by = 8.0 * ps * nX + 12.0 + 8.0 * (double)n_new_max * rec;
        for (int i = 0; i < ne; i++) {
            const GEdge &e = edges[sl.edges[i]];
            spg_edge_ref er;
            er.off = e.off; er.len = e.len; er.kind = e.kind; er.vbegin = 2 * i; er.nv = 2;
            memcpy(&pkt[w], &er, 24);
            w += 3;
            evp[2 * i] = find(sl.verts, nX, e.vtx[0]); evp[2 * i + 1] = find(sl.verts, nX, e.vtx[1]);
            by += 8.0 + 8.0 * e.len;
        }
        alg_bytes += by;
        unsigned long long *dst = port.pkt + (size_t)s * spg::kPktWords;
        memcpy(dst, pkt, (size_t)words * 8);
        port.q->item[(port.tail + (unsigned long long)ahead) % spg::kQCap] = (unsigned long long)(uintptr_t)dst;
    }

    void ring() {
        if (!pending_bell) return;
        P0();
        if (!emulate) {
            std::atomic_thread_fence(std::memory_order_release);
#if defined(__x86_64__)
            __builtin_ia32_sfence();
#endif
            port.tail += (unsigned long long)pending_bell;
            for (int c = 0; c < port.bells; c++) port.q->tail[c * spg::kBellStride] = port.tail;
#if defined(__x86_64__)
            __builtin_ia32_sfence();
#endif
        }
        pending_bell = 0;
        bell_no++;
        g->stats.n_batches++;
        if (helper) hp.launches.store(launch_seq, std::memory_order_release);
        P1(5);
    }

    inline const double *cell(int32_t s) const { return port.h_mail + (size_t)g->sslots[s].mcell * (size_t)port.mail_stride; }

    template <class Pending, class Take>
    inline void scan_mailbox(const uint32_t from, const uint32_t to, const int giveup, Pending &&pending, Take &&take) const {
        const uint32_t mask = (uint32_t)(port.slots - 1);
        int misses = 0;
        for (uint32_t q0 = from; q0 != to && misses < giveup;) {
            const uint32_t nq = std::min<uint32_t>(16, to - q0);
            double w[16];
            for (uint32_t i = 0; i < nq; i++) w[i] = ((const volatile double *)(port.h_mail + (size_t)((q0 + i) & mask) * (size_t)port.mail_stride))[5];
            for (uint32_t i = 0; i < nq; i++) {
                const uint32_t q = q0 + i;
                double tagd;
                const int32_t h = pending(q & mask, tagd);
                if (h < 0) continue;
                const MailState st = mail_state(w[i], tagd);
                if (st != MAIL_NOT_YET) { take(q, h, st == MAIL_FINAL); misses = 0; }
                else misses++;
            }
            q0 += nq;
        }
    }

    void poll_hip(int giveup) {
        std::vector<int32_t> &ready = g->s_ready;
        const uint32_t mask = (uint32_t)(port.slots - 1);
        while (poll_seq != launch_seq && cell_slot[poll_seq & mask] < 0) poll_seq++;
        scan_mailbox(poll_seq, launch_seq, giveup,
                     [&](uint32_t cell, double &tagd) -> int32_t {
                         const int32_t s = cell_slot[cell];
                         if (s >= 0) tagd = (double)g->sslots[s].tag;
                         return s;
                     },
                     [&](uint32_t q, int32_t s, bool) {
                         __builtin_prefetch(&g->sslots[s]); __builtin_prefetch((const char *)&g->sslots[s] + 64); __builtin_prefetch((const char *)&g->sslots[s] + 128);
                         ready.push_back(s);
                         cell_slot[q & mask] = -2;
                     });
        {
            uint32_t q = poll_seq;
            for (int n = 0; q != launch_seq && n < 12; q++) {
                if (cell_slot[q & mask] < 0) continue;
                __builtin_prefetch((const void *)(port.h_mail + (size_t)(q & mask) * (size_t)port.mail_stride));
                n++;
            }
        }
    }

    struct Helper {
        static constexpr uint32_t RQ = 4096;
        alignas(64) std::atomic<uint32_t> launches{0};
        alignas(64) std::atomic<uint32_t> r_tail{0};
        alignas(64) std::atomic<int> stop{0};
        alignas(64) uint32_t r_head = 0;
        std::vector<double> rq;
        std::vector<uint32_t> cell_tag;
        char pad_[64];
    } hp;
    bool helper = false;
    std::thread helper_thread;
    std::vector<const double *> ready_rec;

    void helper_main() {
        const uint32_t mask = (uint32_t)(port.slots - 1);
        std::vector<uint8_t> pend((size_t)port.slots, 0);
        uint32_t head = 0, seen = 0, r_tail = 0;
        unsigned n = 0;
        while (!hp.stop.load(std::memory_order_acquire)) {
            const uint32_t lp = hp.launches.load(std::memory_order_acquire);
            while (seen != lp) { pend[seen & mask] = 1; seen++; }
            while (head != seen && !pend[head & mask]) head++;
            const int giveup = (++n & 15) ? 10 : 1 << 20;
            bool got = false;
            scan_mailbox(head, seen, giveup,
                         [&](uint32_t cell, double &tagd) -> int32_t {
                             if (!pend[cell]) return -1;
                             tagd = (double)hp.cell_tag[cell];
                             return (int32_t)cell;
                         },
                         [&](uint32_t q, int32_t cell, bool final) {
                             double *e = hp.rq.data() + (size_t)(r_tail & (Helper::RQ - 1)) * 8;
                             memcpy(e, port.h_mail + (size_t)cell * (size_t)port.mail_stride, 64);
                             e[5] = (double)(2.0 * (double)q + (final ? 1.0 : 0.0));
                             r_tail++;
                             pend[cell] = 0;
                             got = true;
                         });
            if (got) hp.r_tail.store(r_tail, std::memory_order_release);
        }
    }
    void take_helper_results() {
        const uint32_t rt = hp.r_tail.load(std::memory_order_acquire);
        const uint32_t mask = (uint32_t)(port.slots - 1);
        ready_rec.clear();
        while (hp.r_head != rt) {
            const double *e = hp.rq.data() + (size_t)(hp.r_head & (Helper::RQ - 1)) * 8;
            __builtin_prefetch(e + 8); __builtin_prefetch(e + 16);
            const uint32_t q = (uint32_t)((uint64_t)e[5] >> 1);
            const int32_t s = cell_slot[q & mask];
            g->s_ready.push_back(s);
            ready_rec.push_back(e);
            cell_slot[q & mask] = -2;
            __builtin_prefetch(&g->sslots[s]); __builtin_prefetch((const char *)&g->sslots[s] + 64); __builtin_prefetch((const char *)&g->sslots[s] + 128);
            hp.r_head++;
        }
    }
    bool helper_start() {
#if defined(__linux__)
        static const bool pin = [] { const char *e = getenv("SPG_PIN_THREADS"); return !(e && e[0] == '0'); }();
        if (!pin || sched_getaffinity(0, sizeof old_mask, &old_mask) != 0) return false;
        const int cpu = sched_getcpu();
        int cand = -1;
        for (int d = 1; cpu >= 0 && d < 8 && cand < 0; d++) {
            const int c = (cpu & ~7) | ((cpu + d) & 7);
            if (c < CPU_SETSIZE && CPU_ISSET(c, &old_mask)) cand = c;
        }
        if (cand < 0) return false;
        cpu_set_t one; CPU_ZERO(&one); CPU_SET(cpu, &one);
        if (sched_setaffinity(0, sizeof one, &one) != 0) return false;
        repin = true;
        hp.rq.resize((size_t)Helper::RQ * 8);
        hp.cell_tag.assign((size_t)port.slots, 0);
        helper = true;
        helper_thread = std::thread([this] { helper_main(); });
        CPU_ZERO(&one); CPU_SET(cand, &one);
        (void)pthread_setaffinity_np(helper_thread.native_handle(), sizeof one, &one);
        return true;
#else
        return false;
#endif
    }
    void helper_stop() {
        if (!helper) return;
        hp.stop.store(1, std::memory_order_release);
        helper_thread.join();
        helper = false;
#if defined(__linux__)
        if (repin) (void)sched_setaffinity(0, sizeof old_mask, &old_mask);
#endif
    }
#if defined(__linux__)
    cpu_set_t old_mask;
    bool repin = false;
#endif

    size_t fifo_head = 0;
    uint64_t rng;
    int poll_emulated() {
        std::vector<int32_t> &fifo = g->s_fifo, &ready = g->s_ready;
        std::vector<int32_t> live;
        for (size_t i = fifo_head; i < fifo.size(); i++) if (fifo[i] >= 0) live.push_back((int32_t)i);
        if (live.empty()) { fifo.clear(); fifo_head = 0; return 0; }
        auto next = [&]() { rng ^= rng << 13; rng ^= rng >> 7; rng ^= rng << 17; return rng; };
        size_t take = live.size();
        if (g->stream_emulation > 0) {
            take = 1 + (size_t)(next() % live.size());
            for (size_t i = 0; i + 1 < live.size(); i++) std::swap(live[i], live[i + (size_t)(next() % (live.size() - i))]);
        }
        live.resize(take);
        std::vector<spg_blanket_desc> blk(take);
        std::vector<int64_t> vpo;
        std::vector<spg_edge_ref> er;
        std::vector<int32_t> ev;
        for (size_t t = 0; t < take; t++) {
            const spg_graph::SSlot &sl = g->sslots[fifo[live[t]]];
            spg_blanket_desc &bd = blk[t];
            append_blanket_desc(g, sl.verts, sl.nv, 1, sl.edges, sl.ne, bd, vpo, er, ev);
            bd.n_new_max = sl.n_new_max; bd.n_new_vert_max = 2 * sl.n_new_max;
            bd.new_off = sl.new_off; bd.new_len = (int64_t)sl.n_new_max * rec; bd.out_off = sl.out_off;
        }
        spg_round_desc rd{};
        rd.opts = &g->opts; rd.n_blankets = (int32_t)take; rd.first = 0; rd.count = (int32_t)take;
        rd.blankets = blk.data(); rd.vert_pose_off = vpo.data(); rd.edges = er.data(); rd.edge_vert = ev.data();
        rd.n_vert_total = (int64_t)vpo.size(); rd.n_edge_total = (int64_t)er.size(); rd.n_edge_vert_total = (int64_t)ev.size();
        rd.mail_base = 0; rd.mail_len = 0; rd.slot = 0; rd.tag = ++g->ctx->tag_counter;
        if (int r = g->ctx->be.run_round(g->ctx->be.user, g->dev, &rd)) return r;
        if (int r = g->ctx->be.synchronize(g->ctx->be.user)) return r;
        for (size_t t = 0; t < take; t++) {
            const int32_t s = fifo[live[t]];
            const spg_graph::SSlot &sl = g->sslots[s];
            const int64_t olen = SPG_OUT_LEN(sl.n_new_max, 2 * sl.n_new_max);
            if (int r = g->ctx->be.download(g->ctx->be.user, g->host.data() + sl.out_off, (char *)g->dev + sl.out_off * 8, olen)) return r;
            ready.push_back(s);
            fifo[live[t]] = -1;
        }
        while (fifo_head < fifo.size() && fifo[fifo_head] < 0) fifo_head++;
        return 0;
    }

    std::vector<int32_t> &woken = g->s_woken, &ready = g->s_ready, &fin = g->s_fin;
    size_t fin_head = 0;
    unsigned n_polls = 0;
    uint64_t last_progress = 0, idle_since = 0;

    int take_results() {
        ready.clear();
        P0();
        if (emulate) { if (int r = poll_emulated()) return r; }
        else if (n_inflight) {
            if (helper) take_helper_results(); else poll_hip((++n_polls & 15) ? 10 : 1 << 20);
        }
        P1(0);
        return 0;
    }
    void commit_ready() {
        for (size_t ri = 0; ri < ready.size(); ri++) {
            const int32_t s = ready[ri];
            const double *recd = emulate ? g->host.data() + g->sslots[s].out_off : (helper ? ready_rec[ri] : cell(s));
            const bool fin_now = emulate || (helper ? (((uint64_t)recd[5]) & 1) != 0 : mail_state(recd[5], g->sslots[s].tag) == MAIL_FINAL);
            P0();
            commit(s, recd, fin_now);
            P1(1);
        }
    }
    void examine_woken() {
        if (!fallback) {
            if (woken.size() > 1) std::sort(woken.begin(), woken.end());
            for (size_t wi = 0; wi < woken.size(); wi++) {
                examine(woken[wi]);
                if (pending_bell >= 8) ring();
            }
        }
        woken.clear();
    }
    void late_results() {
        if (emulate || !(fin.size() - fin_head >= 192 || g->s_free.size() < 256 || (cap_wait >= 0 && fin_head < fin.size()))) return;
        P0();
        const size_t n = std::min<size_t>(64, fin.size() - fin_head);
        for (size_t i = 0; i < n; i++) __builtin_prefetch((const void *)cell(fin[fin_head + i]));
        for (size_t i = 0; i < n; i++) {
            const int32_t s = fin[fin_head];
            const volatile double *c = cell(s);
            if (mail_state(c[5], g->sslots[s].tag) != MAIL_FINAL) break;
            harvest(s, (const double *)c);
            fin_head++;
        }
        if (fin_head > 8192) { fin.erase(fin.begin(), fin.begin() + (long)fin_head); fin_head = 0; }
        P1(6);
        if (!woken.empty()) {
            if (!fallback) for (size_t wi = 0; wi < woken.size(); wi++) examine(woken[wi]);
            woken.clear();
        }
    }
    void advance_cursor(const bool got) {
        if (fallback || cursor >= P) return;
        int budget = got ? 4 : 32;
        while (cursor < P && budget-- > 0 && !fallback) {
            examine(cursor++);
            if (!woken.empty()) { for (size_t wi = 0; wi < woken.size() && !fallback; wi++) examine(woken[wi]); woken.clear(); }
        }
    }
    int idle_check() {
        const uint64_t t1 = ticks_now();
        if (!idle_since) idle_since = t1;
        if (n_inflight == 0 && fin_head == fin.size()) {
            fallback = true;
            return 1;
        }
        if (((t1 - last_progress) >> 35) != 0) {
            set_err(g->ctx, SPG_EHIP, "streaming driver: no blanket completed within 10 s");
            return SPG_EHIP;
        }
        return 0;
    }
    int drain() {
        if (!emulate) {
            const double t0 = now_s();
            for (; fin_head < fin.size(); fin_head++) {
                const int32_t s = fin[fin_head];
                const volatile double *c = cell(s);
                uint32_t spins = 0;
                while (mail_state(c[5], g->sslots[s].tag) != MAIL_FINAL) {
                    if ((++spins & 0xfff) == 0 && now_s() - t0 > 10.0) { set_err(g->ctx, SPG_EHIP, "streaming driver: a blanket's KLD tail did not complete within 10 s"); return SPG_EHIP; }
                    cpu_pause();
                }
                harvest(s, (const double *)c);
            }
            woken.clear();
        }
        fin.clear();
        return 0;
    }
    void account(const uint64_t t_begin, const double s_begin) {
        if (idle_since) { t_idle += ticks_now() - idle_since; idle_since = 0; }
        const uint64_t t_end = ticks_now();
        const double secs = now_s() - s_begin;
        const double idle = (t_end > t_begin) ? secs * (double)t_idle / (double)(t_end - t_begin) : 0.0;
        g->stats.device_seconds += idle;
        g->stats.host_seconds += secs - idle;
        g->stats.schedule_seconds += secs - idle;
        if (prof) {
            const char *nm[8] = {"poll", "commit", "examine: parked", "examine: launch decision", "packet", "doorbell", "late results", "launch tail"};
            const double tps = (double)(t_end - t_begin) / secs;
            for (int i = 0; i < 8; i++) fprintf(stderr, "stream prof %-26s %8llu x %8.1f ns = %8.3f ms\n", nm[i], (unsigned long long)pn[i], pn[i] ? 1e9 * (double)pt[i] / tps / (double)pn[i] : 0.0, 1e3 * (double)pt[i] / tps);
        }
    }

    int run() {
        const uint64_t t_begin = ticks_now();
        const double s_begin = now_s();
        last_progress = t_begin;
        for (;;) {
            if (int r = take_results()) return r;
            const bool got = !ready.empty();
            if (got && idle_since) { t_idle += ticks_now() - idle_since; idle_since = 0; }
            commit_ready();
            examine_woken();
            late_results();
            advance_cursor(got);
            ring();
            if (n_done == P) break;
            if (fallback && n_inflight == 0) break;
            if (got || cursor < P) { last_progress = ticks_now(); continue; }
            if (int r = idle_check()) { if (r < 0) return r; break; }
        }
        if (int r = drain()) return r;
        account(t_begin, s_begin);
        return 0;
    }
};
}

int stream_marginalize(spg_graph *g, bool *started) {
    const spg_options &o = g->opts;
    if (started) *started = false;
    static const bool env_off = [] { const char *e = getenv("SPG_STREAM"); return e && e[0] == '0'; }();
    spg::StreamPort *const sim = g->ctx->is_hip ? nullptr : g->ctx->sim_port;
    const bool emulate = !g->ctx->is_hip && !sim;
    if (env_off || g->stream_disabled) return 1;
    if (emulate && g->stream_emulation < 0) return 1;
    if (g->nranks != 1 || o.algorithm != SPG_ALG_NFR || o.topology != SPG_TOPO_TREE || o.lin_point != SPG_LIN_GLOBAL || (o.flags & ~SPG_FLAG_NFR_FACTOR_DESCENT) != 0) return 1;
    const int32_t P = (int32_t)g->pending.size();
    if (P < (emulate ? 1 : 64)) return 1;
    Streamer S(g, emulate);
    if (sim) {
        if (sim->slots < kStreamSlots || sim->mail_stride < kStreamMailStride) return 1;
        S.port = *sim;
    } else if (!emulate) {
        int prc = spg::hip_stream_open(&g->ctx->be, g->d, kStreamSlots, kStreamMailStride, &S.port);
        if (prc < 0) { copy_backend_error(g->ctx); return prc; }
        if (prc > 0) return 1;
    }
    const size_t V = g->vid.size();
    if (g->cst.size() < V) g->cst.resize(V, -1);
    for (int32_t p = 0; p < P; p++) { g->cst[g->pending[p]] = (p << 2) | SV_WAITING; g->vr[g->pending[p]].s.nown = 0; }
    g->wl_next.assign((size_t)P, -1); g->wl_stable.assign((size_t)P, -1); g->wl_done.assign((size_t)P, -1);
    if (g->sslots.size() < (size_t)kStreamSlots) g->sslots.resize(kStreamSlots);
    g->s_free.clear();
    for (int s = kStreamSlots - 1; s >= 0; s--) g->s_free.push_back(s);
    g->s_fifo.clear(); g->s_fin.clear(); g->s_woken.clear(); g->s_ready.clear();
    next_stamp(g);
    if (g->lidx.size() < V) g->lidx.resize(V, -1);
    if ((int64_t)g->host.size() < g->cap) g->host.resize((size_t)g->cap);
    S.rng = 0x9E3779B97F4A7C15ULL ^ ((uint64_t)(g->stream_emulation > 0 ? g->stream_emulation : 1) * 0xD1B54A32D192ED03ULL);
    const int64_t used0 = g->used;
    if (started) *started = true;
    if (g->unsorted_from < 0) g->unsorted_from = (int64_t)g->edges.size();
    if (!emulate) S.cell_slot.assign((size_t)S.port.slots, -1);
    static const int want_helper = [] { const char *e = getenv("SPG_STREAM_THREADS"); return e ? atoi(e) : 0; }();
    if (!emulate && (want_helper == 2 || (want_helper == 0 && !sim)) && P >= 4096) (void)S.helper_start();
    const double t_setup = now_s();
    const int rc = S.run();
    S.helper_stop();
    const double t_ran = now_s();
    if (sim) sim->tail = S.port.tail;
    else if (!emulate) spg::hip_stream_close(&g->ctx->be, &S.port, S.alg_bytes, (long long)S.n_done);
    if (g->used > used0) {
        g->dev_synced = g->used;
        if (!emulate && !sim) mark_stale(g, used0, g->used);
        else {
            if (int r = g->ctx->be.download(g->ctx->be.user, g->host.data() + used0, (char *)g->dev + used0 * 8, g->used - used0)) return r;
        }
    }
    g->stats.n_rounds = S.bell_no;
    g->round_no = S.bell_no;
    size_t left = 0;
    for (int32_t p = 0; p < P; p++) {
        const int32_t v = g->pending[p];
        spg_graph::SVtx &sq = g->vr[v].s;
        const int vst = g->cst[v] & 3;
        if (vst == SV_STABLE) unregister_blanket(g, sq.slot);
        const bool done = vst == SV_DONE;
        g->cst[v] = -1; sq.nown = 0;
        if (!done) g->pending[left++] = v;
    }
    g->pending.resize(left);
    g->pend_head = 0;
    if (getenv("SPG_TRACE")) {
        fprintf(stderr, "spg trace: streaming driver: run %.3f ms, tear-down %.3f ms\n", 1e3 * (t_ran - t_setup), 1e3 * (now_s() - t_ran));
        fprintf(stderr, "spg trace: streaming driver: %d list entries, %d committed in %d doorbells, %zu left to the batch driver (examined up to entry %d)\n",
                P, S.n_done, S.bell_no, left, S.cursor);
        fprintf(stderr, "spg trace: streaming driver: %ld examinations; parked on: earlier neighbour %ld, own blanket %ld, two shared vertices %ld, waiting member of a touching blanket %ld, waiting 2-hop neighbour %ld\n",
                S.n_exam, S.n_park[0], S.n_park[1], S.n_park[2], S.n_park[3], S.n_park[4]);
    }
    if (rc) return rc;
    return left ? 1 : 0;
}

extern "C" int spg_debug_set_stream_port(spg_ctx *c, void *port) {
    if (!c || c->is_hip) return SPG_EINVAL;
    c->sim_port = (spg::StreamPort *)port;
    return 0;
}

extern "C" int spg_graph_set_stream_emulation(spg_graph *g, int seed) {
    if (!g) return SPG_EINVAL;
    g->stream_disabled = seed <= -2;
    g->stream_emulation = seed < 0 ? -1 : seed;
    return 0;
}
```

Before: 3.095 million.

## Persist stream poll helper thread, cache edge data per slot, add lookahead prefetch

The mailbox-polling helper thread now lives on the context and is woken through a condition variable, so it is no longer spawned and joined on every streaming run. Edge key, offset, length and endpoint local indices are cached in a per-examination struct and stored in the slot, so packet building and commit no longer re-read the GEdge records. A sliding prefetch window now covers upcoming pending entries, and stream buffers are pre-reserved during graph setup. Smaller changes add cache-line-aligned slots, validation of result records, perf-counter profiling and integer byte accounting; the extra validation and state add some work per commit.

```diff
diff --git a/sparsifyposegraph_amd/csrc/spg_graph_impl.h b/sparsifyposegraph_amd/csrc/spg_graph_impl.h
--- a/sparsifyposegraph_amd/csrc/spg_graph_impl.h
+++ b/sparsifyposegraph_amd/csrc/spg_graph_impl.h
@@ -119,6 +119,8 @@
     int pcg_max_iter = 0;
     spg_pcg_stats pcg_stats{};
     spg::StreamPort *sim_port = nullptr;
+    struct StreamHelper *stream_helper = nullptr;
+    std::vector<int32_t> stream_cell_slot;
     char err[768] = {0};
 };
 
@@ -253,15 +255,18 @@
     std::vector<double> s_cost;
     std::vector<int> s_first;
     static constexpr int kSOwn = 4, kSMaxV = 16, kSMaxE = 44;
-    struct SSlot {
+    struct alignas(64) SSlot {
         int32_t pos, root, nv, ne, n_new_max, tag, logi, bell;
         int32_t launched;
         int32_t npend, pend[3];
         int32_t mcell;
         int64_t new_off, out_off;
+        uint8_t ends[kSMaxE + 4];
         int32_t verts[kSMaxV];
         int32_t edges[kSMaxE];
     };
+    static_assert(sizeof(SSlot) % 64 == 0 && kSMaxV <= 16, "SSlot: whole cache lines; local vertex indices fit four bits");
+    static constexpr int kSSlotHotLines = 4;
     std::vector<SSlot> sslots;
     std::vector<int32_t> s_free, s_fifo, s_fin, s_woken, s_ready, wl_next, wl_stable, wl_done;
     int64_t unsorted_from = -1;
@@ -291,6 +296,8 @@
 void pose_inverse(int d, const double *a, double *o);
 void quiesce_submission(spg_graph *g);
 int stream_marginalize(spg_graph *g, bool *started = nullptr);
+void stream_reserve(spg_graph *g);
+void stream_ctx_release(spg_ctx *c);
 #pragma GCC visibility pop
 
 namespace {
diff --git a/sparsifyposegraph_amd/csrc/spg_host.cpp b/sparsifyposegraph_amd/csrc/spg_host.cpp
--- a/sparsifyposegraph_amd/csrc/spg_host.cpp
+++ b/sparsifyposegraph_amd/csrc/spg_host.cpp
@@ -122,6 +122,7 @@
 
 extern "C" void spg_ctx_destroy(spg_ctx *c) {
     if (!c) return;
+    stream_ctx_release(c);
     if (c->rccl) spg::rccl_comm_destroy(c->rccl);
     if (c->is_hip) spg::hip_backend_destroy(&c->be);
     delete c;
@@ -466,6 +467,7 @@
         touch(g->owners, 8192); touch(g->ocnt, 8192); touch(g->owner_free, 8192); touch(g->transient, 4096); touch(g->Dpool, 65536);
         touch(g->s_newpending, 4096); touch(g->hdr_buf, 65536);
     }
+    stream_reserve(g);
     return sync_device(g);
 }
 
diff --git a/sparsifyposegraph_amd/csrc/spg_host_stream.cpp b/sparsifyposegraph_amd/csrc/spg_host_stream.cpp
--- a/sparsifyposegraph_amd/csrc/spg_host_stream.cpp
+++ b/sparsifyposegraph_amd/csrc/spg_host_stream.cpp
@@ -1,4 +1,11 @@
 #include "spg_graph_impl.h"
+#include <condition_variable>
+#include <mutex>
+#if defined(__linux__)
+#include <linux/perf_event.h>
+#include <sys/ioctl.h>
+#include <sys/syscall.h>
+#endif
 
 #if defined(__x86_64__)
 #include <x86intrin.h>
@@ -7,6 +14,28 @@
 static inline uint64_t ticks_now() { return (uint64_t)(now_s() * 1e9); }
 #endif
 
+struct StreamHelper {
+    static constexpr uint32_t RQ = 4096;
+    alignas(64) std::atomic<uint32_t> launches{0};
+    alignas(64) std::atomic<uint32_t> r_tail{0};
+    alignas(64) std::atomic<int> stop{0};
+    alignas(64) std::atomic<int> busy{0};
+    alignas(64) uint32_t r_head = 0;
+    std::vector<double> rq;
+    std::vector<uint32_t> cell_tag;
+    alignas(64) const double *h_mail = nullptr;
+    int mail_stride = 0, slots = 0;
+    std::vector<uint8_t> pend;
+    std::mutex m;
+    std::condition_variable cv;
+    uint64_t job = 0;
+    bool quit = false;
+    int cpu = -1;
+    pid_t pid = 0;
+    std::thread th;
+    char pad_[64];
+};
+
 namespace {
 enum : uint8_t { SV_WAITING = 0, SV_STABLE = 1, SV_INFLIGHT = 2, SV_DONE = 3 };
 constexpr int kStreamSlots = 2048;
@@ -18,6 +47,73 @@
     for (int i = 0; i < sl.nv; i++) {
         spg_graph::SVtx &sx = vr[sl.verts[i]].s;
         for (int j = 0; j < sx.nown; j++) if (sx.own[j] == s) { sx.own[j] = sx.own[--sx.nown]; break; }
+    }
+}
+
+template <class Pending, class Take>
+inline void scan_mailbox_cells(const double *const h_mail, const int mail_stride, const int slots, const uint32_t from, const uint32_t to,
+                               const int giveup, Pending &&pending, Take &&take) {
+    const uint32_t mask = (uint32_t)(slots - 1);
+    int misses = 0;
+    for (uint32_t q0 = from; q0 != to && misses < giveup;) {
+        const uint32_t nq = std::min<uint32_t>(16, to - q0);
+        double w[16];
+        for (uint32_t i = 0; i < nq; i++) w[i] = ((const volatile double *)(h_mail + (size_t)((q0 + i) & mask) * (size_t)mail_stride))[5];
+        for (uint32_t i = 0; i < nq; i++) {
+            const uint32_t q = q0 + i;
+            double tagd;
+            const int32_t h = pending(q & mask, tagd);
+            if (h < 0) continue;
+            const MailState st = mail_state(w[i], tagd);
+            if (st != MAIL_NOT_YET) { take(q, h, st == MAIL_FINAL); misses = 0; }
+            else misses++;
+        }
+        q0 += nq;
+    }
+}
+
+void stream_helper_serve(StreamHelper &hp) {
+    const double *const h_mail = hp.h_mail;
+    const int mail_stride = hp.mail_stride, slots = hp.slots;
+    const uint32_t mask = (uint32_t)(slots - 1);
+    std::vector<uint8_t> &pend = hp.pend;
+    pend.assign((size_t)slots, 0);
+    uint32_t head = 0, seen = 0, r_tail = 0;
+    unsigned n = 0;
+    while (!hp.stop.load(std::memory_order_acquire)) {
+        const uint32_t lp = hp.launches.load(std::memory_order_acquire);
+        while (seen != lp) { pend[seen & mask] = 1; seen++; }
+        while (head != seen && !pend[head & mask]) head++;
+        const int giveup = (++n & 15) ? 10 : 1 << 20;
+        bool got = false;
+        scan_mailbox_cells(h_mail, mail_stride, slots, head, seen, giveup,
+                           [&](uint32_t cell, double &tagd) -> int32_t {
+                               if (!pend[cell]) return -1;
+                               tagd = (double)hp.cell_tag[cell];
+                               return (int32_t)cell;
+                           },
+                           [&](uint32_t q, int32_t cell, bool final) {
+                               double *e = hp.rq.data() + (size_t)(r_tail & (StreamHelper::RQ - 1)) * 8;
+                               memcpy(e, h_mail + (size_t)cell * (size_t)mail_stride, 64);
+                               e[5] = (double)(2.0 * (double)q + (final ? 1.0 : 0.0));
+                               r_tail++;
+                               pend[cell] = 0;
+                               got = true;
+                           });
+        if (got) hp.r_tail.store(r_tail, std::memory_order_release);
+    }
+}
+void stream_helper_thread(StreamHelper *hp) {
+    uint64_t served = 0;
+    for (;;) {
+        {
+            std::unique_lock<std::mutex> lk(hp->m);
+            hp->cv.wait(lk, [&] { return hp->quit || hp->job != served; });
+            if (hp->quit) return;
+            served = hp->job;
+        }
+        stream_helper_serve(*hp);
+        hp->busy.store(0, std::memory_order_release);
     }
 }
 
@@ -34,12 +130,44 @@
     uint64_t t_idle = 0;
 
     Streamer(spg_graph *g_, bool emu) : g(g_), emulate(emu), D(g_->d), ps(g_->ps), rec(g_->rec), P((int32_t)g_->pending.size()), arena_dev(g_->dev) {}
-
+    ~Streamer() { counters_close(); }
+
+    struct BEdge { int64_t key, off; int32_t eid, len; int8_t kind; uint8_t la, lb; };
     struct SvView { spg_graph::VRec *vr; spg_graph::SVtx &operator[](int32_t i) const { return vr[i].s; } };
 
     long n_exam = 0, n_park[8] = {0};
     const bool prof = [] { const char *e = getenv("SPG_STREAM_PROF"); return e && e[0] == '1'; }();
     uint64_t pt[8] = {0}, pn[8] = {0}, pt_last = 0;
+    int pc_fd[2] = {-1, -1};
+    void counters_open() {
+#if defined(__linux__)
+        const uint64_t what[2] = {PERF_COUNT_HW_CPU_CYCLES, PERF_COUNT_HW_INSTRUCTIONS};
+        for (int i = 0; i < 2; i++) {
+            struct perf_event_attr pa;
+            memset(&pa, 0, sizeof pa);
+            pa.type = PERF_TYPE_HARDWARE; pa.size = sizeof pa; pa.config = what[i];
+            pa.disabled = i == 0; pa.exclude_kernel = 1; pa.exclude_hv = 1; pa.read_format = PERF_FORMAT_GROUP;
+            pc_fd[i] = (int)syscall(SYS_perf_event_open, &pa, 0, -1, i ? pc_fd[0] : -1, 0);
+            if (pc_fd[i] < 0) { counters_close(); return; }
+        }
+        ioctl(pc_fd[0], PERF_EVENT_IOC_RESET, PERF_IOC_FLAG_GROUP);
+        ioctl(pc_fd[0], PERF_EVENT_IOC_ENABLE, PERF_IOC_FLAG_GROUP);
+#endif
+    }
+    void counters_close() {
+        for (int i = 1; i >= 0; i--) if (pc_fd[i] >= 0) { close(pc_fd[i]); pc_fd[i] = -1; }
+    }
+    void counters_report() {
+        uint64_t buf[3] = {0, 0, 0};
+        if (pc_fd[0] < 0 || read(pc_fd[0], buf, sizeof buf) != (ssize_t)sizeof buf || buf[0] != 2) {
+            fprintf(stderr, "stream prof counters unavailable\n");
+        } else {
+            const double n = (double)std::max(n_done, 1);
+            fprintf(stderr, "stream prof counters: %.0f cycles, %.0f instructions per removed vertex (user space, graph thread), IPC %.2f\n",
+                    (double)buf[1] / n, (double)buf[2] / n, buf[1] ? (double)buf[2] / (double)buf[1] : 0.0);
+        }
+        counters_close();
+    }
     inline void P0() { if (prof) pt_last = ticks_now(); }
     inline void P1(int i) { if (prof) { const uint64_t n = ticks_now(); pt[i] += n - pt_last; pn[i]++; pt_last = n; } }
     void park(std::vector<int32_t> &heads, int32_t on, int32_t p) { g->wl_next[p] = heads[on]; heads[on] = p; }
@@ -77,6 +205,26 @@
         sl.ne = 0; sl.launched = 0; sl.logi = -1;
         g->cst[v] = (p << 2) | SV_STABLE; sv[v].slot = s;
         if (g->wl_stable[p] >= 0) wake(g->wl_stable, p);
+    }
+
+    static constexpr int kPfDist = 512, kPfLead = 16;
+    inline void prefetch_entry(const int32_t p) const {
+        const spg_graph::VRec *const vr = g->vr.data();
+        const GEdge *const edges = g->edges.data();
+        const int32_t v = g->pending[p];
+        __builtin_prefetch((const char *)&vr[v] + 64);
+        for (const spg_graph::AdjEnt &a : vr[v].adj) {
+            __builtin_prefetch(&edges[a.eid]);
+            __builtin_prefetch(&vr[a.other]);
+            __builtin_prefetch((const char *)&vr[a.other] + 64);
+        }
+    }
+    void prefetch_ahead() {
+        const int32_t to = std::min<int32_t>(P, n_done + n_inflight + kPfDist);
+        for (; prefetched_to < to; prefetched_to++) {
+            if (prefetched_to + kPfLead < P) __builtin_prefetch(&g->vr[g->pending[prefetched_to + kPfLead]]);
+            prefetch_entry(prefetched_to);
+        }
     }
 
     int examine(const int32_t p) {
@@ -122,15 +270,6 @@
             if (blocker >= 0) {
                 n_park[0]++;
                 park(g->wl_done, blocker, p);
-                if (p >= prefetched_to) {
-                    prefetched_to = p + 1;
-                    __builtin_prefetch((const char *)&vr[v] + 64);
-                    for (const spg_graph::AdjEnt &a : vr[v].adj) {
-                        __builtin_prefetch(&edges[a.eid]);
-                        __builtin_prefetch(&vr[a.other]);
-                        __builtin_prefetch((const char *)&vr[a.other] + 64);
-                    }
-                }
                 return 0;
             }
             for (int i = 2; i < nX; i++) {
@@ -168,7 +307,7 @@
             }
             if (blocker >= 0) { n_park[3]++; reserve(p, X, nX); park(g->wl_done, blocker, p); return 0; }
         }
-        int32_t E[spg_graph::kSMaxE];
+        BEdge E[spg_graph::kSMaxE];
         int ne = 0;
         for (int i = 1; i < nX; i++) {
             for (const spg_graph::AdjEnt &a : vr[X[i]].adj) {
@@ -178,7 +317,8 @@
                 if (j >= 0) {
                     if (j == 0 || j >= i) {
                         if (ne == spg_graph::kSMaxE) { fallback = true; return 0; }
-                        E[ne++] = a.eid;
+                        E[ne].eid = a.eid; E[ne].la = (uint8_t)i; E[ne].lb = (uint8_t)j;
+                        ne++;
                     }
                 } else {
                     const int32_t c = cst[y];
@@ -196,11 +336,17 @@
         const int n_new_max = k - 1, n_new_vert_max = 2 * (k - 1);
         const int64_t new_len = (int64_t)n_new_max * rec, out_len = emulate ? SPG_OUT_LEN(n_new_max, n_new_vert_max) : 0;
         if (g->used + new_len + out_len > g->cap) { fallback = true; return 0; }
+        for (int i = 0; i < ne; i++) {
+            BEdge &b = E[i];
+            const GEdge &e = edges[b.eid];
+            b.key = e.key; b.off = e.off; b.len = e.len; b.kind = e.kind;
+            if (e.vtx[0] != X[b.la]) std::swap(b.la, b.lb);
+        }
         for (int i = 1; i < ne; i++) {
-            const int32_t eid = E[i]; const int64_t key = edges[eid].key;
+            const BEdge b = E[i];
             int j = i - 1;
-            for (; j >= 0 && edges[E[j]].key > key; j--) E[j + 1] = E[j];
-            E[j + 1] = eid;
+            for (; j >= 0 && E[j].key > b.key; j--) E[j + 1] = E[j];
+            E[j + 1] = b;
         }
         int32_t s = mine;
         if (s < 0) { s = g->s_free.back(); g->s_free.pop_back(); }
@@ -213,11 +359,11 @@
         sl.out_off = emulate ? g->used : -1;
         sl.new_off = g->used + out_len;
         g->used += new_len + out_len;
-        memcpy(sl.edges, E, sizeof(int32_t) * (size_t)ne);
+        for (int i = 0; i < ne; i++) { sl.edges[i] = E[i].eid; sl.ends[i] = (uint8_t)(E[i].la | (E[i].lb << 4)); }
         cst[v] = (p << 2) | SV_INFLIGHT; sv[v].slot = s;
         P1(3);
-        if (!emulate) build_packet(s, pending_bell);
-        if (helper) hp.cell_tag[sl.mcell] = (uint32_t)sl.tag;
+        if (!emulate) build_packet(s, E, pending_bell);
+        if (helper) hpp->cell_tag[sl.mcell] = (uint32_t)sl.tag;
         P1(4);
         pending_bell++;
         n_inflight++;
@@ -226,10 +372,19 @@
         return 1;
     }
 
-    void commit(const int32_t s, const double *recd, const bool final_seen) {
+    inline bool compact_record_ok(const spg_graph::SSlot &sl, const double *recd) const {
+        if (!(recd[4] >= 0 && recd[4] <= (double)sl.n_new_max && recd[0] >= SPG_OK && recd[0] <= SPG_ST_NEEDS_LOCAL_OPTIMIZATION)) return false;
+        bool ok = true;
+        for_each_compact_edge(recd, (int)recd[4], [&](int, int la, int lb) { ok &= la < sl.nv && lb < sl.nv && la != lb; });
+        return ok;
+    }
+    int commit(const int32_t s, const double *recd, const bool final_seen) {
         spg_graph::SSlot &sl = g->sslots[s];
         const int32_t p = sl.pos, v = sl.root;
+        if (!emulate && !compact_record_ok(sl, recd))
+            return set_err(g->ctx, SPG_EHIP, "streaming driver: malformed result record for vertex %s", std::to_string(g->vid[v]).c_str());
         const int status = (int)recd[0], inf = (int)recd[1], n_new = (int)recd[4];
+        spg_graph::VRec *const vr = g->vr.data();
         sl.logi = (int32_t)g->log.size();
         g->log.push_back({g->vid[v], sl.bell, status, inf, recd[2], recd[3]});
         g->stats.max_blanket = std::max(g->stats.max_blanket, sl.nv);
@@ -238,10 +393,10 @@
         else {
             for (int i = 0; i < sl.ne; i++) {
                 const int32_t eid = sl.edges[i];
-                GEdge &e = g->edges[eid];
-                e.alive = 0;
-                adj_remove(g->vr[e.vtx[0]].adj, eid);
-                if (e.vtx[1] != e.vtx[0]) adj_remove(g->vr[e.vtx[1]].adj, eid);
+                const int la = sl.ends[i] & 15, lb = sl.ends[i] >> 4;
+                g->edges[eid].alive = 0;
+                adj_remove(vr[sl.verts[la]].adj, eid);
+                if (lb != la) adj_remove(vr[sl.verts[lb]].adj, eid);
             }
             g->n_mutations += sl.ne + 1;
             g->n_live_e -= sl.ne;
@@ -276,6 +431,7 @@
         if (final_seen) harvest(s, recd);
         else g->s_fin.push_back(s);
         if (g->wl_done[p] >= 0) wake(g->wl_done, p);
+        return 0;
     }
     void harvest(const int32_t s, const double *recd) {
         spg_graph::SSlot &sl = g->sslots[s];
@@ -292,13 +448,12 @@
     void *arena_dev;
     static_assert(sizeof(spg::StreamPort) + sizeof(void *) == 64, "port + arena_dev = the cache line the poll helper reads");
     uint32_t launch_seq = 0, poll_seq = 0;
-    std::vector<int32_t> cell_slot;
-    double alg_bytes = 0;
-
-    void build_packet(const int32_t s, const int ahead) {
+    std::vector<int32_t> &cell_slot = g->ctx->stream_cell_slot;
+    int64_t alg_bytes = 0;
+
+    void build_packet(const int32_t s, const BEdge *E, const int ahead) {
         const spg_graph::SSlot &sl = g->sslots[s];
         const spg_graph::VRec *const vr = g->vr.data();
-        const GEdge *const edges = g->edges.data();
         const int nX = sl.nv, ne = sl.ne, n_new_max = sl.n_new_max;
         const int words = spg::kPktHdr + nX + 4 * ne;
         unsigned long long pkt[spg::kPktWords];
@@ -315,15 +470,15 @@
         int w = spg::kPktHdr;
         for (int i = 0; i < nX; i++) pkt[w++] = (unsigned long long)vr[sl.verts[i]].pose;
         int32_t *evp = (int32_t *)(pkt + spg::kPktHdr + nX + 3 * ne);
-        double by = 8.0 * ps * nX + 12.0 + 8.0 * (double)n_new_max * rec;
+        int64_t by = 8 * (int64_t)ps * nX + 12 + 8 * (int64_t)n_new_max * rec;
         for (int i = 0; i < ne; i++) {
-            const GEdge &e = edges[sl.edges[i]];
+            const BEdge &e = E[i];
             spg_edge_ref er;
             er.off = e.off; er.len = e.len; er.kind = e.kind; er.vbegin = 2 * i; er.nv = 2;
             memcpy(&pkt[w], &er, 24);
             w += 3;
-            evp[2 * i] = find(sl.verts, nX, e.vtx[0]); evp[2 * i + 1] = find(sl.verts, nX, e.vtx[1]);
-            by += 8.0 + 8.0 * e.len;
+            evp[2 * i] = e.la; evp[2 * i + 1] = e.lb;
+            by += 8 + 8 * (int64_t)e.len;
         }
         alg_bytes += by;
         unsigned long long *dst = port.pkt + (size_t)s * spg::kPktWords;
@@ -348,7 +503,7 @@
         pending_bell = 0;
         bell_no++;
         g->stats.n_batches++;
-        if (helper) hp.launches.store(launch_seq, std::memory_order_release);
+        if (helper) hpp->launches.store(launch_seq, std::memory_order_release);
         P1(5);
     }
 
@@ -356,23 +511,7 @@
 
     template <class Pending, class Take>
     inline void scan_mailbox(const uint32_t from, const uint32_t to, const int giveup, Pending &&pending, Take &&take) const {
-        const uint32_t mask = (uint32_t)(port.slots - 1);
-        int misses = 0;
-        for (uint32_t q0 = from; q0 != to && misses < giveup;) {
-            const uint32_t nq = std::min<uint32_t>(16, to - q0);
-            double w[16];
-            for (uint32_t i = 0; i < nq; i++) w[i] = ((const volatile double *)(port.h_mail + (size_t)((q0 + i) & mask) * (size_t)port.mail_stride))[5];
-            for (uint32_t i = 0; i < nq; i++) {
-                const uint32_t q = q0 + i;
-                double tagd;
-                const int32_t h = pending(q & mask, tagd);
-                if (h < 0) continue;
-                const MailState st = mail_state(w[i], tagd);
-                if (st != MAIL_NOT_YET) { take(q, h, st == MAIL_FINAL); misses = 0; }
-                else misses++;
-            }
-            q0 += nq;
-        }
+        scan_mailbox_cells(port.h_mail, port.mail_stride, port.slots, from, to, giveup, pending, take);
     }
 
     void poll_hip(int giveup) {
@@ -386,7 +525,7 @@
                          return s;
                      },
                      [&](uint32_t q, int32_t s, bool) {
-                         __builtin_prefetch(&g->sslots[s]); __builtin_prefetch((const char *)&g->sslots[s] + 64); __builtin_prefetch((const char *)&g->sslots[s] + 128);
+                         prefetch_slot(s);
                          ready.push_back(s);
                          cell_slot[q & mask] = -2;
                      });
@@ -400,61 +539,28 @@
         }
     }
 
-    struct Helper {
-        static constexpr uint32_t RQ = 4096;
-        alignas(64) std::atomic<uint32_t> launches{0};
-        alignas(64) std::atomic<uint32_t> r_tail{0};
-        alignas(64) std::atomic<int> stop{0};
-        alignas(64) uint32_t r_head = 0;
-        std::vector<double> rq;
-        std::vector<uint32_t> cell_tag;
-        char pad_[64];
-    } hp;
+    StreamHelper *hpp = nullptr;
     bool helper = false;
-    std::thread helper_thread;
     std::vector<const double *> ready_rec;
 
-    void helper_main() {
-        const uint32_t mask = (uint32_t)(port.slots - 1);
-        std::vector<uint8_t> pend((size_t)port.slots, 0);
-        uint32_t head = 0, seen = 0, r_tail = 0;
-        unsigned n = 0;
-        while (!hp.stop.load(std::memory_order_acquire)) {
-            const uint32_t lp = hp.launches.load(std::memory_order_acquire);
-            while (seen != lp) { pend[seen & mask] = 1; seen++; }
-            while (head != seen && !pend[head & mask]) head++;
-            const int giveup = (++n & 15) ? 10 : 1 << 20;
-            bool got = false;
-            scan_mailbox(head, seen, giveup,
-                         [&](uint32_t cell, double &tagd) -> int32_t {
-                             if (!pend[cell]) return -1;
-                             tagd = (double)hp.cell_tag[cell];
-                             return (int32_t)cell;
-                         },
-                         [&](uint32_t q, int32_t cell, bool final) {
-                             double *e = hp.rq.data() + (size_t)(r_tail & (Helper::RQ - 1)) * 8;
-                             memcpy(e, port.h_mail + (size_t)cell * (size_t)port.mail_stride, 64);
-                             e[5] = (double)(2.0 * (double)q + (final ? 1.0 : 0.0));
-                             r_tail++;
-                             pend[cell] = 0;
-                             got = true;
-                         });
-            if (got) hp.r_tail.store(r_tail, std::memory_order_release);
-        }
+    inline void prefetch_slot(const int32_t s) const {
+        const char *const c = (const char *)&g->sslots[s];
+        for (int l = 0; l < spg_graph::kSSlotHotLines; l++) __builtin_prefetch(c + 64 * l);
     }
     void take_helper_results() {
+        StreamHelper &hp = *hpp;
         const uint32_t rt = hp.r_tail.load(std::memory_order_acquire);
         const uint32_t mask = (uint32_t)(port.slots - 1);
         ready_rec.clear();
         while (hp.r_head != rt) {
-            const double *e = hp.rq.data() + (size_t)(hp.r_head & (Helper::RQ - 1)) * 8;
+            const double *e = hp.rq.data() + (size_t)(hp.r_head & (StreamHelper::RQ - 1)) * 8;
             __builtin_prefetch(e + 8); __builtin_prefetch(e + 16);
             const uint32_t q = (uint32_t)((uint64_t)e[5] >> 1);
             const int32_t s = cell_slot[q & mask];
             g->s_ready.push_back(s);
             ready_rec.push_back(e);
             cell_slot[q & mask] = -2;
-            __builtin_prefetch(&g->sslots[s]); __builtin_prefetch((const char *)&g->sslots[s] + 64); __builtin_prefetch((const char *)&g->sslots[s] + 128);
+            prefetch_slot(s);
             hp.r_head++;
         }
     }
@@ -472,24 +578,43 @@
         cpu_set_t one; CPU_ZERO(&one); CPU_SET(cpu, &one);
         if (sched_setaffinity(0, sizeof one, &one) != 0) return false;
         repin = true;
-        hp.rq.resize((size_t)Helper::RQ * 8);
+        spg_ctx *const c = g->ctx;
+        if (c->stream_helper && c->stream_helper->pid != getpid()) c->stream_helper = nullptr;
+        if (!c->stream_helper) {
+            c->stream_helper = new StreamHelper;
+            c->stream_helper->pid = getpid();
+            c->stream_helper->rq.resize((size_t)StreamHelper::RQ * 8);
+            c->stream_helper->th = std::thread(stream_helper_thread, c->stream_helper);
+        }
+        StreamHelper &hp = *c->stream_helper;
+        hpp = &hp;
+        if (hp.cpu != cand) {
+            CPU_ZERO(&one); CPU_SET(cand, &one);
+            (void)pthread_setaffinity_np(hp.th.native_handle(), sizeof one, &one);
+            hp.cpu = cand;
+        }
         hp.cell_tag.assign((size_t)port.slots, 0);
+        hp.h_mail = port.h_mail; hp.mail_stride = port.mail_stride; hp.slots = port.slots;
+        hp.r_head = 0;
+        hp.launches.store(0, std::memory_order_relaxed); hp.r_tail.store(0, std::memory_order_relaxed);
+        hp.stop.store(0, std::memory_order_relaxed); hp.busy.store(1, std::memory_order_relaxed);
+        { std::lock_guard<std::mutex> lk(hp.m); hp.job++; }
+        hp.cv.notify_one();
         helper = true;
-        helper_thread = std::thread([this] { helper_main(); });
-        CPU_ZERO(&one); CPU_SET(cand, &one);
-        (void)pthread_setaffinity_np(helper_thread.native_handle(), sizeof one, &one);
         return true;
 #else
         return false;
 #endif
     }
     void helper_stop() {
-        if (!helper) return;
-        hp.stop.store(1, std::memory_order_release);
-        helper_thread.join();
-        helper = false;
+        if (helper) {
+            hpp->stop.store(1, std::memory_order_release);
+            uint32_t spins = 0;
+            while (hpp->busy.load(std::memory_order_acquire)) spin_wait(spins);
+            helper = false;
+        }
 #if defined(__linux__)
-        if (repin) (void)sched_setaffinity(0, sizeof old_mask, &old_mask);
+        if (repin) { (void)sched_setaffinity(0, sizeof old_mask, &old_mask); repin = false; }
 #endif
     }
 #if defined(__linux__)
@@ -556,15 +681,17 @@
         P1(0);
         return 0;
     }
-    void commit_ready() {
+    int commit_ready() {
         for (size_t ri = 0; ri < ready.size(); ri++) {
             const int32_t s = ready[ri];
             const double *recd = emulate ? g->host.data() + g->sslots[s].out_off : (helper ? ready_rec[ri] : cell(s));
             const bool fin_now = emulate || (helper ? (((uint64_t)recd[5]) & 1) != 0 : mail_state(recd[5], g->sslots[s].tag) == MAIL_FINAL);
             P0();
-            commit(s, recd, fin_now);
+            const int rc = commit(s, recd, fin_now);
             P1(1);
-        }
+            if (rc) return rc;
+        }
+        return 0;
     }
     void examine_woken() {
         if (!fallback) {
@@ -645,6 +772,8 @@
         if (prof) {
             const char *nm[8] = {"poll", "commit", "examine: parked", "examine: launch decision", "packet", "doorbell", "late results", "launch tail"};
             const double tps = (double)(t_end - t_begin) / secs;
+            fprintf(stderr, "stream prof %d removed in %.3f ms busy + %.3f ms waiting = %.1f ns per removed vertex\n", n_done, 1e3 * (secs - idle), 1e3 * idle, 1e9 * (secs - idle) / (double)std::max(n_done, 1));
+            counters_report();
             for (int i = 0; i < 8; i++) fprintf(stderr, "stream prof %-26s %8llu x %8.1f ns = %8.3f ms\n", nm[i], (unsigned long long)pn[i], pn[i] ? 1e9 * (double)pt[i] / tps / (double)pn[i] : 0.0, 1e3 * (double)pt[i] / tps);
         }
     }
@@ -653,14 +782,16 @@
         const uint64_t t_begin = ticks_now();
         const double s_begin = now_s();
         last_progress = t_begin;
+        if (prof) counters_open();
         for (;;) {
             if (int r = take_results()) return r;
             const bool got = !ready.empty();
             if (got && idle_since) { t_idle += ticks_now() - idle_since; idle_since = 0; }
-            commit_ready();
+            if (int r = commit_ready()) return r;
             examine_woken();
             late_results();
             advance_cursor(got);
+            prefetch_ahead();
             ring();
             if (n_done == P) break;
             if (fallback && n_inflight == 0) break;
@@ -674,10 +805,15 @@
 };
 }
 
+static bool stream_env_off() {
+    static const bool off = [] { const char *e = getenv("SPG_STREAM"); return e && e[0] == '0'; }();
+    return off;
+}
+
 int stream_marginalize(spg_graph *g, bool *started) {
     const spg_options &o = g->opts;
     if (started) *started = false;
-    static const bool env_off = [] { const char *e = getenv("SPG_STREAM"); return e && e[0] == '0'; }();
+    const bool env_off = stream_env_off();
     spg::StreamPort *const sim = g->ctx->is_hip ? nullptr : g->ctx->sim_port;
     const bool emulate = !g->ctx->is_hip && !sim;
     if (env_off || g->stream_disabled) return 1;
@@ -696,14 +832,13 @@
     }
     const size_t V = g->vid.size();
     if (g->cst.size() < V) g->cst.resize(V, -1);
-    for (int32_t p = 0; p < P; p++) { g->cst[g->pending[p]] = (p << 2) | SV_WAITING; g->vr[g->pending[p]].s.nown = 0; }
+    for (int32_t p = 0; p < P; p++) g->cst[g->pending[p]] = (p << 2) | SV_WAITING;
     g->wl_next.assign((size_t)P, -1); g->wl_stable.assign((size_t)P, -1); g->wl_done.assign((size_t)P, -1);
     if (g->sslots.size() < (size_t)kStreamSlots) g->sslots.resize(kStreamSlots);
     g->s_free.clear();
     for (int s = kStreamSlots - 1; s >= 0; s--) g->s_free.push_back(s);
     g->s_fifo.clear(); g->s_fin.clear(); g->s_woken.clear(); g->s_ready.clear();
-    next_stamp(g);
-    if (g->lidx.size() < V) g->lidx.resize(V, -1);
+    if (emulate && g->lidx.size() < V) g->lidx.resize(V, -1);
     if ((int64_t)g->host.size() < g->cap) g->host.resize((size_t)g->cap);
     S.rng = 0x9E3779B97F4A7C15ULL ^ ((uint64_t)(g->stream_emulation > 0 ? g->stream_emulation : 1) * 0xD1B54A32D192ED03ULL);
     const int64_t used0 = g->used;
@@ -713,11 +848,12 @@
     static const int want_helper = [] { const char *e = getenv("SPG_STREAM_THREADS"); return e ? atoi(e) : 0; }();
     if (!emulate && (want_helper == 2 || (want_helper == 0 && !sim)) && P >= 4096) (void)S.helper_start();
     const double t_setup = now_s();
+    const bool helper_on = S.helper;
     const int rc = S.run();
     S.helper_stop();
     const double t_ran = now_s();
     if (sim) sim->tail = S.port.tail;
-    else if (!emulate) spg::hip_stream_close(&g->ctx->be, &S.port, S.alg_bytes, (long long)S.n_done);
+    else if (!emulate) spg::hip_stream_close(&g->ctx->be, &S.port, (double)S.alg_bytes, (long long)S.n_done);
     if (g->used > used0) {
         g->dev_synced = g->used;
         if (!emulate && !sim) mark_stale(g, used0, g->used);
@@ -730,17 +866,16 @@
     size_t left = 0;
     for (int32_t p = 0; p < P; p++) {
         const int32_t v = g->pending[p];
-        spg_graph::SVtx &sq = g->vr[v].s;
         const int vst = g->cst[v] & 3;
-        if (vst == SV_STABLE) unregister_blanket(g, sq.slot);
-        const bool done = vst == SV_DONE;
-        g->cst[v] = -1; sq.nown = 0;
-        if (!done) g->pending[left++] = v;
+        if (vst == SV_STABLE) unregister_blanket(g, g->vr[v].s.slot);
+        g->cst[v] = -1;
+        if (vst != SV_DONE) g->pending[left++] = v;
     }
     g->pending.resize(left);
     g->pend_head = 0;
+    if (rc) for (spg_graph::VRec &r : g->vr) r.s.nown = 0;
     if (getenv("SPG_TRACE")) {
-        fprintf(stderr, "spg trace: streaming driver: run %.3f ms, tear-down %.3f ms\n", 1e3 * (t_ran - t_setup), 1e3 * (now_s() - t_ran));
+        fprintf(stderr, "spg trace: streaming driver: run %.3f ms, tear-down %.3f ms, poll helper %s\n", 1e3 * (t_ran - t_setup), 1e3 * (now_s() - t_ran), helper_on ? "on" : "off");
         fprintf(stderr, "spg trace: streaming driver: %d list entries, %d committed in %d doorbells, %zu left to the batch driver (examined up to entry %d)\n",
                 P, S.n_done, S.bell_no, left, S.cursor);
         fprintf(stderr, "spg trace: streaming driver: %ld examinations; parked on: earlier neighbour %ld, own blanket %ld, two shared vertices %ld, waiting member of a touching blanket %ld, waiting 2-hop neighbour %ld\n",
@@ -748,6 +883,28 @@
     }
     if (rc) return rc;
     return left ? 1 : 0;
+}
+
+void stream_reserve(spg_graph *g) {
+    if (stream_env_off() || g->stream_disabled || g->nranks != 1 || (!g->ctx->is_hip && !g->ctx->sim_port && g->stream_emulation < 0)) return;
+    const size_t V = g->vid.size();
+    auto touch = [](auto &v, size_t n) { if (v.capacity() < n) { const size_t keep = v.size(); v.resize(n); v.resize(keep); } };
+    if (g->cst.size() < V) g->cst.resize(V, -1);
+    touch(g->wl_next, V); touch(g->wl_stable, V); touch(g->wl_done, V);
+    if (g->sslots.size() < (size_t)kStreamSlots) g->sslots.resize(kStreamSlots);
+    touch(g->s_free, kStreamSlots); touch(g->s_fin, 16384); touch(g->s_woken, 4096); touch(g->s_ready, 4096);
+    touch(g->ctx->stream_cell_slot, kStreamSlots);
+}
+
+void stream_ctx_release(spg_ctx *c) {
+    StreamHelper *const hp = c->stream_helper;
+    if (!hp) return;
+    c->stream_helper = nullptr;
+    if (hp->pid != getpid()) return;
+    { std::lock_guard<std::mutex> lk(hp->m); hp->quit = true; }
+    hp->cv.notify_one();
+    hp->th.join();
+    delete hp;
 }
 
 extern "C" int spg_debug_set_stream_port(spg_ctx *c, void *port) {
```

Result: faster. 3.328 million, median of 6 (+7.5%).
